# trifectatechfoundation/zlib-rs

Measured on NVIDIA H100. Metric: deflate_level6_raw_input_throughput_silesia_small_tar, higher is better.
Workload: dtype u8

## Files before the change

include/zb_engine.h:

```cpp
#ifndef ZB_ENGINE_H
#define ZB_ENGINE_H
#include <stddef.h>
#include <stdint.h>

#ifdef __cplusplus
extern "C" {
#endif

#define ZB_API __attribute__((visibility("default")))

#define ZB_OK 0
#define ZB_E_NODEVICE (-100)
#define ZB_E_CUDA (-101)
#define ZB_E_BUF (-5)
#define ZB_E_MEM (-4)
#define ZB_E_PARAM (-2)
#define ZB_E_DATA (-3)
#define ZB_E_INTERNAL (-102)

typedef struct zb_engine zb_engine;

typedef struct zb_deflate_result {
    uint64_t out_bytes;
    uint32_t check;
    int32_t data_type;
    uint32_t iterations;
    uint32_t n_symbols;
    uint32_t n_blocks;
    uint32_t gpu_launches;
    int32_t exact_parity;
    float gpu_ms;
    uint32_t bits_used;
    uint32_t carry;
} zb_deflate_result;

ZB_API zb_engine *zb_engine_create(int device, int *err);
ZB_API void zb_engine_destroy(zb_engine *e);
ZB_API const char *zb_last_error(void);
ZB_API int zb_device_count(void);

ZB_API int zb_deflate(zb_engine *e, const void *src, size_t src_len, int src_on_device, void *dst, size_t dst_cap, int dst_on_device,
               int level, int strategy, int window_bits, zb_deflate_result *res);
#define ZB_FLAG_NOT_LAST 1u
#define ZB_FLAG_LOW_PARALLEL 2u
#define ZB_FLAG_CHECK_ADLER 4u
#define ZB_FLAG_CHECK_CRC 8u
#define ZB_FLAG_END_PARTIAL 16u
#define ZB_FLAG_END_BLOCK 32u
#define ZB_FLAG_PRIME(bits, val) ((((uint32_t)(bits) & 7u) << 12) | (((uint32_t)(val) & 0xffu) << 16))
#define ZB_FLAG_MEMLEVEL(m) ((uint32_t)(m) << 8)
ZB_API int zb_deflate_ex(zb_engine *e, const void *src, size_t src_len, int src_on_device, void *dst, size_t dst_cap, int dst_on_device,
                  int level, int strategy, int window_bits, uint32_t flags, zb_deflate_result *res);
ZB_API int zb_deflate_dict(zb_engine *e, const void *dict, size_t dict_len, const void *src, size_t src_len, int src_on_device, void *dst,
                           size_t dst_cap, int dst_on_device, int level, int strategy, int window_bits, uint32_t flags, zb_deflate_result *res);
ZB_API size_t zb_deflate_bound(size_t src_len);

typedef struct zb_inflate_result {
    uint64_t out_bytes;
    uint64_t in_bytes;
    uint32_t check;
    int32_t status;
    uint32_t gpu_launches;
    float gpu_ms;
    char msg[64];
} zb_inflate_result;

ZB_API int zb_inflate(zb_engine *e, const void *src, size_t src_len, int src_on_device, void *dst, size_t dst_cap, int dst_on_device,
               int window_bits, zb_inflate_result *res);

#define ZB_INF_CHECK_ADLER 1u
#define ZB_INF_CHECK_CRC 2u
ZB_API int zb_inflate_ex(zb_engine *e, const void *src, size_t src_len, int src_on_device, void *dst, size_t dst_cap, int dst_on_device,
                         int window_bits, uint32_t flags, zb_inflate_result *res);

typedef struct zb_inflate_seg {
    uint64_t out_bytes;
    uint64_t end_bit;
    uint32_t final_block, need_input, sync_point;
    uint32_t check;
    uint32_t gpu_launches;
    float gpu_ms;
    char msg[64];
} zb_inflate_seg;
ZB_API int zb_inflate_blocks(zb_engine *e, const void *src, size_t src_len, uint64_t start_bit, const void *dict, size_t dict_len,
                             void *dst, size_t dst_cap, int check_kind, uint32_t check_start, zb_inflate_seg *out);

ZB_API int zb_adler32(zb_engine *e, uint32_t start, const void *buf, size_t len, int on_device, uint32_t *out, float *gpu_ms);
ZB_API int zb_crc32(zb_engine *e, uint32_t start, const void *buf, size_t len, int on_device, uint32_t *out, float *gpu_ms);

ZB_API void zb_engine_set_profile(zb_engine *e, int on);
ZB_API int zb_engine_get_profile(zb_engine *e, float *ms, uint32_t *launches, int n);

ZB_API void *zb_device_alloc(zb_engine *e, size_t bytes);
ZB_API void zb_device_free(zb_engine *e, void *p);
ZB_API int zb_copy_to_device(zb_engine *e, void *dst, const void *src, size_t bytes);
ZB_API int zb_copy_to_host(zb_engine *e, void *dst, const void *src, size_t bytes);
ZB_API int zb_device_fill_random(zb_engine *e, void *dst, size_t bytes, uint64_t seed);

#ifdef __cplusplus
}
#endif
#endif
```

zlib_rs_b200/__init__.py:

```python
import ctypes
import os

_HERE = os.path.dirname(os.path.abspath(__file__))
LIB_PATH = os.environ.get("ZB_LIB_PATH") or os.path.join(_HERE, "libz_b200.so")

Z_OK, Z_STREAM_END, Z_NEED_DICT = 0, 1, 2
Z_ERRNO, Z_STREAM_ERROR, Z_DATA_ERROR, Z_MEM_ERROR, Z_BUF_ERROR, Z_VERSION_ERROR = -1, -2, -3, -4, -5, -6
Z_NO_FLUSH, Z_PARTIAL_FLUSH, Z_SYNC_FLUSH, Z_FULL_FLUSH, Z_FINISH, Z_BLOCK = 0, 1, 2, 3, 4, 5
Z_DEFAULT_STRATEGY, Z_FILTERED, Z_HUFFMAN_ONLY, Z_RLE, Z_FIXED = 0, 1, 2, 3, 4
ZLIB_VERSION = b"1.3.0-zlib-rs-0.6.7-b200"
ZB_FLAG_NOT_LAST = 1
ZB_FLAG_LOW_PARALLEL = 2
ZB_FLAG_CHECK_ADLER = 4
ZB_FLAG_CHECK_CRC = 8


class ZStream(ctypes.Structure):
    _fields_ = [("next_in", ctypes.c_void_p), ("avail_in", ctypes.c_uint), ("total_in", ctypes.c_ulong),
                ("next_out", ctypes.c_void_p), ("avail_out", ctypes.c_uint), ("total_out", ctypes.c_ulong),
                ("msg", ctypes.c_char_p), ("state", ctypes.c_void_p), ("zalloc", ctypes.c_void_p),
                ("zfree", ctypes.c_void_p), ("opaque", ctypes.c_void_p), ("data_type", ctypes.c_int),
                ("adler", ctypes.c_ulong), ("reserved", ctypes.c_ulong)]


class DeflateResult(ctypes.Structure):
    _fields_ = [("out_bytes", ctypes.c_uint64), ("check", ctypes.c_uint32), ("data_type", ctypes.c_int32),
                ("iterations", ctypes.c_uint32), ("n_symbols", ctypes.c_uint32), ("n_blocks", ctypes.c_uint32),
                ("gpu_launches", ctypes.c_uint32), ("exact_parity", ctypes.c_int32), ("gpu_ms", ctypes.c_float),
                ("bits_used", ctypes.c_uint32), ("carry", ctypes.c_uint32)]


class InflateResult(ctypes.Structure):
    _fields_ = [("out_bytes", ctypes.c_uint64), ("in_bytes", ctypes.c_uint64), ("check", ctypes.c_uint32),
                ("status", ctypes.c_int32), ("gpu_launches", ctypes.c_uint32), ("gpu_ms", ctypes.c_float),
                ("msg", ctypes.c_char * 64)]


class ZlibError(Exception):
    def __init__(self, code, msg=""):
        super().__init__("zlib error %d %s" % (code, msg))
        self.code = code
        self.msg = msg


_lib = None


def lib():
    global _lib
    if _lib is None:
        if not os.path.exists(LIB_PATH):
            raise RuntimeError("libz_b200.so is not built: run `python -c 'import __graft_entry__ as g; g.build()'` "
                               "or `make -C zlib_rs_b200/csrc` (needs nvcc, sm_90a)")
        L = ctypes.CDLL(LIB_PATH, mode=ctypes.RTLD_LOCAL)
        vp, sz, u32, u64, ci = ctypes.c_void_p, ctypes.c_size_t, ctypes.c_uint32, ctypes.c_uint64, ctypes.c_int
        ul = ctypes.c_ulong
        zs = ctypes.POINTER(ZStream)
        L.zlibVersion.restype = ctypes.c_char_p
        L.zError.restype, L.zError.argtypes = ctypes.c_char_p, [ci]
        L.deflateInit2_.argtypes = [zs, ci, ci, ci, ci, ci, ctypes.c_char_p, ci]
        L.deflateInit_.argtypes = [zs, ci, ctypes.c_char_p, ci]
        L.deflate.argtypes = [zs, ci]
        L.deflateEnd.argtypes = [zs]
        L.deflateReset.argtypes = [zs]
        L.deflateBound.argtypes, L.deflateBound.restype = [zs, ul], ul
        L.inflateInit2_.argtypes = [zs, ci, ctypes.c_char_p, ci]
        L.inflateInit_.argtypes = [zs, ctypes.c_char_p, ci]
        L.inflate.argtypes = [zs, ci]
        L.inflateEnd.argtypes = [zs]
        L.compress2.argtypes = [vp, ctypes.POINTER(ul), vp, ul, ci]
        L.compress.argtypes = [vp, ctypes.POINTER(ul), vp, ul]
        L.compressBound.argtypes, L.compressBound.restype = [ul], ul
        L.uncompress.argtypes = [vp, ctypes.POINTER(ul), vp, ul]
        L.uncompress2.argtypes = [vp, ctypes.POINTER(ul), vp, ctypes.POINTER(ul)]
        for f in ("adler32", "crc32"):
            getattr(L, f).argtypes, getattr(L, f).restype = [ul, vp, ctypes.c_uint], ul
            getattr(L, f + "_z").argtypes, getattr(L, f + "_z").restype = [ul, vp, sz], ul
        L.adler32_combine.argtypes, L.adler32_combine.restype = [ul, ul, ctypes.c_long], ul
        L.crc32_combine.argtypes, L.crc32_combine.restype = [ul, ul, ctypes.c_long], ul
        L.crc32_combine_gen.argtypes, L.crc32_combine_gen.restype = [ctypes.c_long], ul
        L.adler32_combine64.argtypes, L.adler32_combine64.restype = [ul, ul, ctypes.c_longlong], ul
        L.crc32_combine64.argtypes, L.crc32_combine64.restype = [ul, ul, ctypes.c_longlong], ul
        L.crc32_combine_gen64.argtypes, L.crc32_combine_gen64.restype = [ctypes.c_longlong], ul
        L.crc32_combine_op.argtypes, L.crc32_combine_op.restype = [ul, ul, ul], ul
        L.zb_engine_create.argtypes, L.zb_engine_create.restype = [ci, ctypes.POINTER(ci)], vp
        L.zb_engine_destroy.argtypes = [vp]
        L.zb_last_error.restype = ctypes.c_char_p
        L.zb_device_count.restype = ci
        L.zb_deflate.argtypes = [vp, vp, sz, ci, vp, sz, ci, ci, ci, ci, ctypes.POINTER(DeflateResult)]
        L.zb_deflate_ex.argtypes = [vp, vp, sz, ci, vp, sz, ci, ci, ci, ci, u32, ctypes.POINTER(DeflateResult)]
        L.zb_deflate_bound.argtypes, L.zb_deflate_bound.restype = [sz], sz
        L.zb_inflate.argtypes = [vp, vp, sz, ci, vp, sz, ci, ci, ctypes.POINTER(InflateResult)]
        L.zb_adler32.argtypes = [vp, u32, vp, sz, ci, ctypes.POINTER(u32), ctypes.POINTER(ctypes.c_float)]
        L.zb_crc32.argtypes = [vp, u32, vp, sz, ci, ctypes.POINTER(u32), ctypes.POINTER(ctypes.c_float)]
        L.zb_engine_set_profile.argtypes = [vp, ci]
        L.zb_engine_get_profile.argtypes = [vp, ctypes.POINTER(ctypes.c_float), ctypes.POINTER(u32), ci]
        L.zb_device_alloc.argtypes, L.zb_device_alloc.restype = [vp, sz], vp
        L.zb_device_free.argtypes = [vp, vp]
        L.zb_copy_to_device.argtypes = [vp, vp, vp, sz]
        L.zb_copy_to_host.argtypes = [vp, vp, vp, sz]
        L.zb_device_fill_random.argtypes = [vp, vp, sz, u64]
        _lib = L
    return _lib


def _buf(data):
    data = bytes(data)
    return data, (ctypes.c_char * max(len(data), 1)).from_buffer_copy(data or b"\0")


def compressBound(n):
    return lib().compressBound(n)


def compress2(data, level=-1):
    data, src = _buf(data)
    n = ctypes.c_ulong(lib().compressBound(len(data)))
    dst = ctypes.create_string_buffer(n.value)
    rc = lib().compress2(dst, ctypes.byref(n), src, len(data), level)
    if rc != Z_OK:
        raise ZlibError(rc, lib().zb_last_error().decode())
    return dst.raw[: n.value]


def compress(data):
    return compress2(data, -1)


def uncompress(data, bufsize):
    data, src = _buf(data)
    n = ctypes.c_ulong(bufsize)
    dst = ctypes.create_string_buffer(max(bufsize, 1))
    rc = lib().uncompress(dst, ctypes.byref(n), src, len(data))
    if rc != Z_OK:
        raise ZlibError(rc, lib().zb_last_error().decode())
    return dst.raw[: n.value]


def crc32(data, value=0):
    data, src = _buf(data)
    return lib().crc32_z(value, src if data else None, len(data)) if data else (value if True else 0)


def adler32(data, value=1):
    data, src = _buf(data)
    return lib().adler32_z(value, src, len(data)) if data else value


class Deflate:

    def __init__(self, level=-1, window_bits=15, mem_level=8, strategy=0):
        self.s = ZStream()
        rc = lib().deflateInit2_(ctypes.byref(self.s), level, 8, window_bits, mem_level, strategy, ZLIB_VERSION,
                                 ctypes.sizeof(ZStream))
        if rc != Z_OK:
            raise ZlibError(rc, (self.s.msg or b"").decode())
        self._open = True

    def deflate(self, data, flush=Z_NO_FLUSH, out_chunk=1 << 16):
        data, src = _buf(data)
        self.s.next_in = ctypes.addressof(src)
        self.s.avail_in = len(data)
        out = bytearray()
        obuf = ctypes.create_string_buffer(out_chunk)
        while True:
            self.s.next_out = ctypes.addressof(obuf)
            self.s.avail_out = out_chunk
            rc = lib().deflate(ctypes.byref(self.s), flush)
            out += obuf.raw[: out_chunk - self.s.avail_out]
            if rc == Z_STREAM_END:
                break
            if rc == Z_BUF_ERROR and self.s.avail_in == 0:
                break
            if rc != Z_OK:
                raise ZlibError(rc, (self.s.msg or b"").decode())
            if self.s.avail_out != 0 and self.s.avail_in == 0:
                break
        self.last_rc = rc
        return bytes(out)

    @property
    def adler(self):
        return self.s.adler

    @property
    def total_in(self):
        return self.s.total_in

    @property
    def total_out(self):
        return self.s.total_out

    @property
    def data_type(self):
        return self.s.data_type

    def end(self):
        if self._open:
            self._open = False
            return lib().deflateEnd(ctypes.byref(self.s))
        return Z_OK

    def __del__(self):
        try:
            self.end()
        except Exception:
            pass


class Inflate:

    def __init__(self, window_bits=15):
        self.s = ZStream()
        rc = lib().inflateInit2_(ctypes.byref(self.s), window_bits, ZLIB_VERSION, ctypes.sizeof(ZStream))
        if rc != Z_OK:
            raise ZlibError(rc, (self.s.msg or b"").decode())
        self._open = True
        self.eof = False

    def inflate(self, data, flush=Z_NO_FLUSH, out_chunk=1 << 16):
        data, src = _buf(data)
        self.s.next_in = ctypes.addressof(src)
        self.s.avail_in = len(data)
        out = bytearray()
        obuf = ctypes.create_string_buffer(out_chunk)
        while True:
            self.s.next_out = ctypes.addressof(obuf)
            self.s.avail_out = out_chunk
            rc = lib().inflate(ctypes.byref(self.s), flush)
            out += obuf.raw[: out_chunk - self.s.avail_out]
            if rc == Z_STREAM_END:
                self.eof = True
                break
            if rc == Z_BUF_ERROR:
                break
            if rc != Z_OK:
                raise ZlibError(rc, (self.s.msg or b"").decode())
            if self.s.avail_out != 0 and self.s.avail_in == 0:
                break
        self.last_rc = rc
        return bytes(out)

    @property
    def adler(self):
        return self.s.adler

    def end(self):
        if self._open:
            self._open = False
            return lib().inflateEnd(ctypes.byref(self.s))
        return Z_OK

    def __del__(self):
        try:
            self.end()
        except Exception:
            pass


class Engine:
    def __init__(self, device=0):
        err = ctypes.c_int(0)
        self.h = lib().zb_engine_create(device, ctypes.byref(err))
        if not self.h:
            raise RuntimeError("zb_engine_create failed (%d): %s" % (err.value, lib().zb_last_error().decode()))

    def close(self):
        if self.h:
            lib().zb_engine_destroy(self.h)
            self.h = None

    def __del__(self):
        try:
            self.close()
        except Exception:
            pass

    def _check(self, rc):
        if rc != 0:
            raise ZlibError(rc, lib().zb_last_error().decode())

    def alloc(self, n):
        p = lib().zb_device_alloc(self.h, n)
        if not p:
            raise MemoryError("zb_device_alloc(%d)" % n)
        return p

    def free(self, p):
        lib().zb_device_free(self.h, p)

    def to_device(self, dptr, data):
        data, src = _buf(data)
        self._check(lib().zb_copy_to_device(self.h, dptr, src, len(data)))

    def to_host(self, dptr, n):
        dst = ctypes.create_string_buffer(max(n, 1))
        self._check(lib().zb_copy_to_host(self.h, dst, dptr, n))
        return dst.raw[:n]

    def deflate(self, src, n=None, level=6, strategy=0, window_bits=15, flags=0, src_on_device=False, dst=None, dst_cap=0,
                dst_on_device=False, mem_level=8):
        res = DeflateResult()
        flags |= (mem_level & 15) << 8
        keep = None
        if not src_on_device:
            data, keep = _buf(src)
            n = len(data)
            src = ctypes.addressof(keep)
        own = None
        if dst is None:
            dst_cap = lib().zb_deflate_bound(n) + 64
            own = ctypes.create_string_buffer(dst_cap)
            dst = ctypes.addressof(own)
            dst_on_device = False
        rc = lib().zb_deflate_ex(self.h, src, n, int(src_on_device), dst, dst_cap, int(dst_on_device), level, strategy,
                                 window_bits, flags, ctypes.byref(res))
        self._check(rc)
        return (own.raw[: res.out_bytes] if own is not None else None), res

    def inflate(self, src, out_cap, n=None, window_bits=15, src_on_device=False, dst=None, dst_on_device=False):
        res = InflateResult()
        keep = None
        if not src_on_device:
            data, keep = _buf(src)
            n = len(data)
            src = ctypes.addressof(keep)
        own = None
        if dst is None:
            own = ctypes.create_string_buffer(max(out_cap, 1))
            dst = ctypes.addressof(own)
        rc = lib().zb_inflate(self.h, src, n, int(src_on_device), dst, out_cap, int(dst_on_device), window_bits, ctypes.byref(res))
        return rc, (own.raw[: res.out_bytes] if own is not None else None), res

    def adler32(self, buf, n=None, start=1, on_device=False):
        out, ms = ctypes.c_uint32(0), ctypes.c_float(0)
        keep = None
        if not on_device:
            data, keep = _buf(buf)
            n = len(data)
            buf = ctypes.addressof(keep)
        self._check(lib().zb_adler32(self.h, start, buf, n, int(on_device), ctypes.byref(out), ctypes.byref(ms)))
        return out.value, ms.value

    def crc32(self, buf, n=None, start=0, on_device=False):
        out, ms = ctypes.c_uint32(0), ctypes.c_float(0)
        keep = None
        if not on_device:
            data, keep = _buf(buf)
            n = len(data)
            buf = ctypes.addressof(keep)
        self._check(lib().zb_crc32(self.h, start, buf, n, int(on_device), ctypes.byref(out), ctypes.byref(ms)))
        return out.value, ms.value

    PHASES = ["links", "match", "nxt", "path", "emit_holes", "tail", "blocks", "encode", "checksum", "h2d", "d2h", "match_first"]

    def set_profile(self, on=True):
        lib().zb_engine_set_profile(self.h, int(on))

    def get_profile(self):
        ms = (ctypes.c_float * 12)()
        ln = (ctypes.c_uint32 * 12)()
        k = lib().zb_engine_get_profile(self.h, ms, ln, 12)
        return {self.PHASES[i]: {"ms": ms[i], "launches": ln[i]} for i in range(min(k, len(self.PHASES)))}

    def fill_random(self, dptr, n, seed=42):
        self._check(lib().zb_device_fill_random(self.h, dptr, n, seed))
```

zlib_rs_b200/csrc/zb_engine.cu:

```cuda
#include <cuda_runtime.h>
#include <stdio.h>
#include <stdlib.h>
#include <string.h>
#include <new>
#include "../../include/zb_engine.h"
#include "zb_kernels.cuh"
#include "zb_engine_internal.h"

namespace zb {

constexpr uint32_t kSlowSub9 = 24576;
constexpr uint32_t kTailTiles = 2;
constexpr uint32_t kTailSub = 512;

thread_local char g_err[256] = "";

static void set_err(const char *what, cudaError_t e)
{
    snprintf(g_err, sizeof g_err, "%s: %s", what, cudaGetErrorString(e));
}

#define CK(call)                                                  \
    do {                                                          \
        cudaError_t e_ = (call);                                  \
        if (e_ != cudaSuccess) { set_err(#call, e_); return ZB_E_CUDA; } \
    } while (0)

__global__ void k_match(JobBufs);
__global__ void k_skip(JobBufs);
__global__ void k_nxt(JobBufs);
__global__ void k_path_tiles(JobBufs);
__global__ void k_path_chain(JobBufs, uint32_t, uint32_t);
__global__ void k_path_groups(JobBufs, uint32_t, uint32_t, uint4 *, uint32_t *);
__global__ void k_path_chain2(JobBufs, uint32_t, uint32_t, const uint4 *, uint32_t *, uint32_t *);
__global__ void k_path_mark(JobBufs, const uint32_t *, const uint32_t *);
__global__ void k_iter_lists(JobBufs, uint32_t *, uint32_t *, uint32_t);
__global__ void k_emit(JobBufs);
__global__ void k_holes(JobBufs, uint32_t);
__global__ void k_holes_cmp(JobBufs, uint32_t, uint32_t);
__global__ void k_tail(JobBufs);
__global__ void k_block_hist(JobBufs, uint32_t *);
__global__ void k_build_blocks(JobBufs, const uint32_t *);
__global__ void k_scan_blocks(JobBufs);
__global__ void k_encode(JobBufs);
__global__ void k_finish(JobBufs, const uint32_t *);
__global__ void k_literal_syms(JobBufs);
__global__ void k_stored(JobBufs);
__global__ void k_links2_std(JobBufs, uint32_t);
__global__ void k_links2_roll(JobBufs, uint32_t);
__global__ void k_links_fix_std(JobBufs);
__global__ void k_links_fix_roll(JobBufs);
__global__ void k_slow(JobBufs);
__global__ void k_rle(JobBufs);
__global__ void k_emit_slow(JobBufs);
__global__ void k_tail_slow(JobBufs);
__global__ void k_serial_low(JobBufs);
__global__ void k_links_dict_ghost(JobBufs, uint32_t *);
__global__ void k_links_dict_ghost_apply(JobBufs, const uint32_t *);

constexpr uint32_t kMatchSmemBytes = (kWSize + kMatchSub + 512) + (kWSize + kMatchSub) * 2 + ((kWSize + kMatchSub) / 32 + 1) * 4 * 4 + 8192;
constexpr uint32_t kPathSmemBytes = kPathTile * 4 * 3;
constexpr uint32_t kLinks2SmemBytes = 65536 * 2 + kLinkTile * 2 + kLinkTile + 64 + 2048;
constexpr uint32_t kSkipSmemBytes = 2 * kWSize * 2 + 2 * (2 * kWSize / 32) * 4 + 8192 + 64;
constexpr uint32_t kSlowSubMax = 24576;
constexpr uint32_t kSlowSmemBytes = (kWSize + kSlowSubMax + kSlowAhead) * 3;
constexpr uint32_t kChainSmemBytes = kChainChunkTiles * kPathHead * 8;
constexpr uint32_t kChain2MaxSmem = 200 * 1024;
constexpr uint32_t kSerialSmemBytes = (65536 + kWSize) * 2 + 35824 + 16;
constexpr uint32_t kSerialSmemQuick = 65536 * 2 + 65536 + 16;

int Engine::init(int dev)
{
    int n = 0;
    cudaError_t e = cudaGetDeviceCount(&n);
    if (e != cudaSuccess || n == 0) {
        snprintf(g_err, sizeof g_err, "no CUDA device (%s)", e == cudaSuccess ? "count 0" : cudaGetErrorString(e));
        return ZB_E_NODEVICE;
    }
    if (dev < 0 || dev >= n) { snprintf(g_err, sizeof g_err, "device %d out of range", dev); return ZB_E_PARAM; }
    device = dev;
    CK(cudaSetDevice(dev));
    CK(cudaStreamCreateWithFlags(&st, cudaStreamNonBlocking));
    CK(cudaStreamCreateWithFlags(&st2, cudaStreamNonBlocking));
    CK(cudaEventCreateWithFlags(&evf, cudaEventDisableTiming));
    CK(cudaEventCreateWithFlags(&evt, cudaEventDisableTiming));
    for (int i = 0; i < kUpChunks; i++) CK(cudaEventCreateWithFlags(&evc[i], cudaEventDisableTiming));
    CK(cudaEventCreateWithFlags(&evk, cudaEventDisableTiming));
    CK(cudaEventCreate(&ev0));
    CK(cudaEventCreate(&ev1));
    CK(upload_tables());
    CK(cudaFuncSetAttribute(k_match, cudaFuncAttributeMaxDynamicSharedMemorySize, kMatchSmemBytes));
    CK(cudaFuncSetAttribute(k_skip, cudaFuncAttributeMaxDynamicSharedMemorySize, kSkipSmemBytes));
    CK(cudaFuncSetAttribute(k_links2_std, cudaFuncAttributeMaxDynamicSharedMemorySize, kLinks2SmemBytes));
    CK(cudaFuncSetAttribute(k_links2_roll, cudaFuncAttributeMaxDynamicSharedMemorySize, kLinks2SmemBytes));
    CK(cudaFuncSetAttribute(k_slow, cudaFuncAttributeMaxDynamicSharedMemorySize, kSlowSmemBytes));
    CK(cudaFuncSetAttribute(k_path_tiles, cudaFuncAttributeMaxDynamicSharedMemorySize, kPathSmemBytes));
    CK(cudaFuncSetAttribute(k_path_mark, cudaFuncAttributeMaxDynamicSharedMemorySize, kPathSmemBytes));
    CK(cudaFuncSetAttribute(k_path_chain, cudaFuncAttributeMaxDynamicSharedMemorySize, kChainSmemBytes));
    CK(cudaFuncSetAttribute(k_path_groups, cudaFuncAttributeMaxDynamicSharedMemorySize, kChain2MaxSmem));
    CK(cudaFuncSetAttribute(k_path_chain2, cudaFuncAttributeMaxDynamicSharedMemorySize, kChain2MaxSmem));
    CK(cudaFuncSetAttribute(k_serial_low, cudaFuncAttributeMaxDynamicSharedMemorySize, kSerialSmemBytes));
    CK(cudaMallocHost(&h_info, sizeof(JobInfo)));
    CK(cudaMalloc(&d_info, sizeof(JobInfo)));
    CK(cudaMalloc(&d_check, 16));
    { int rc_ = inflate_init(); if (rc_ != ZB_OK) return rc_; }
    return ZB_OK;
}

Engine::~Engine()
{
    if (device < 0) return;
    cudaSetDevice(device);
    for (auto &b : bufs) if (b.p) cudaFree(b.p);
    if (h_stage) cudaFreeHost(h_stage);
    if (h_info) cudaFreeHost(h_info);
    if (d_info) cudaFree(d_info);
    if (d_check) cudaFree(d_check);
    if (ev0) cudaEventDestroy(ev0);
    if (ev1) cudaEventDestroy(ev1);
    if (evf) cudaEventDestroy(evf);
    if (evt) cudaEventDestroy(evt);
    for (int i = 0; i < kUpChunks; i++) if (evc[i]) cudaEventDestroy(evc[i]);
    if (evk) cudaEventDestroy(evk);
    if (st2) cudaStreamDestroy(st2);
    if (st) cudaStreamDestroy(st);
}

void Engine::pbegin()
{
    if (!profile) return;
    if (!pev0) { cudaEventCreate(&pev0); cudaEventCreate(&pev1); }
    cudaEventRecord(pev0, st);
}

void Engine::pend(int phase, uint32_t nlaunch)
{
    if (!profile) return;
    cudaEventRecord(pev1, st);
    cudaEventSynchronize(pev1);
    float ms = 0;
    cudaEventElapsedTime(&ms, pev0, pev1);
    phase_ms[phase] += ms;
    phase_launches[phase] += nlaunch;
}

int Engine::reserve(int slot, size_t bytes, void **out)
{
    Buf &b = bufs[slot];
    if (b.cap < bytes) {
        if (b.p) { cudaFree(b.p); b.p = nullptr; b.cap = 0; }
        size_t want = bytes + (bytes >> 3) + 4096;
        cudaError_t e = cudaMalloc(&b.p, want);
        if (e != cudaSuccess) { set_err("cudaMalloc", e); return ZB_E_MEM; }
        b.cap = want;
    }
    *out = b.p;
    return ZB_OK;
}

int Engine::stage(size_t bytes)
{
    if (h_stage_cap < bytes) {
        if (h_stage) cudaFreeHost(h_stage);
        h_stage = nullptr;
        h_stage_cap = 0;
        cudaError_t e = cudaMallocHost(&h_stage, bytes + (bytes >> 3) + 4096);
        if (e != cudaSuccess) { set_err("cudaMallocHost", e); return ZB_E_MEM; }
        h_stage_cap = bytes + (bytes >> 3) + 4096;
    }
    return ZB_OK;
}

enum { S_IN, S_L, S_HOLES, S_HOLESN, S_M, S_NXT, S_PEXIT, S_PCNT, S_SYMIDX, S_TENTRY, S_TSYMB, S_TDIRTY, S_SYMS, S_SYMB,
       S_BLOCKS, S_SCRATCH, S_FREQ, S_OUT, S_CK, S_INF0, S_INF1, S_PHEAD, S_SK, S_MARKN, S_LLIST, S_LCNT, S_BMAP, S_HDIFF, S_HCOARSE, S_CSTATE, S_LISTS, S_LR, S_LLAST, S_BBASE, S_MCHG, S_GFN, S_KEYS, S_COUNT };
static_assert(S_COUNT <= Engine::kSlots, "slots");

size_t deflate_bound(size_t n)
{
    return n + ((n + 7) >> 3) + ((n + 63) >> 6) + 5 + 18 + 64;
}

int Engine::deflate(const void *src, size_t n_in, bool src_dev, void *dst, size_t dst_cap, bool dst_dev, int level, int strategy,
                    int window_bits, uint32_t flags, zb_deflate_result *res, const void *dict, size_t dict_len)
{
    size_t dstart = 0;
    if (dict_len) {
        if (!dict || window_bits >= 0) { snprintf(g_err, sizeof g_err, "a dictionary needs a raw stream (the caller frames FDICT / DICTID)"); return ZB_E_PARAM; }
        if (dict_len >= 2 * (size_t)kWSize) { dict = static_cast<const uint8_t *>(dict) + (dict_len - kWSize); dict_len = kWSize; }
        dstart = dict_len;
    }
    const size_t n = n_in + dstart;
    int mem_level = (int)((flags >> 8) & 15u);
    if (mem_level == 0) mem_level = 8;
    if (mem_level > 9) return ZB_E_PARAM;
    if (!res || (!src && n) || !dst) return ZB_E_PARAM;
    memset(res, 0, sizeof *res);
    if (n > 0xF0000000ull) { snprintf(g_err, sizeof g_err, "input too large for one job (%zu)", n); return ZB_E_PARAM; }
    if (level == -1) level = 6;
    if (level < 0 || level > 9 || strategy < 0 || strategy > 4) return ZB_E_PARAM;
    uint32_t wrap;
    if (window_bits < 0) { if (window_bits < -15 || window_bits > -8) return ZB_E_PARAM; wrap = 0; }
    else if (window_bits > 15) { if (window_bits < 24 || window_bits > 31) return ZB_E_PARAM; wrap = 2; }
    else { if (window_bits < 8) return ZB_E_PARAM; wrap = 1; }
    const int wb = window_bits < 0 ? -window_bits : window_bits > 15 ? window_bits - 16 : window_bits;
    CK(cudaSetDevice(device));
    const uint32_t N = (uint32_t)n;
    launches = 0;

    JobBufs jb;
    memset(&jb, 0, sizeof jb);
    int rc;
    void *p;
    const size_t npad = (size_t)N + kPad;
    const uint32_t nwords = (N >> 5) + 2;
    const uint32_t nmt = N / kMatchTile + 1, npt = N / kPathTile + 1;
    const bool low_parallel = (flags & ZB_FLAG_LOW_PARALLEL) != 0 || dstart != 0;
    const bool serial_low = (level == 1 || level == 2) && strategy != 2 && strategy != 3 && !low_parallel;
    const uint32_t block_syms = (serial_low && level == 1) ? kBlockSyms : (1u << (mem_level + 6)) - 1u;
    const uint32_t max_blocks = N / block_syms + 2;
    const size_t out_cap = (deflate_bound(n) + 15) & ~(size_t)15;
    if ((rc = stage((size_t)nmt + 64 + ((size_t)N / 512 + 2 + npt + nmt + 8) * 4 + 64)) != ZB_OK) return rc;
    uint8_t *h_dirty = static_cast<uint8_t *>(h_stage);
    uint32_t *h_lists = reinterpret_cast<uint32_t *>(static_cast<uint8_t *>(h_stage) + (((size_t)nmt + 64 + 15) & ~(size_t)15));
#define RES(slot, bytes, field, type)                                   \
    if ((rc = reserve(slot, bytes, &p)) != ZB_OK) return rc;            \
    jb.field = static_cast<type>(p);
    uint8_t *d_in;
    if ((rc = reserve(S_IN, npad + 16, &p)) != ZB_OK) return rc;
    d_in = static_cast<uint8_t *>(p);
    jb.in = d_in;
    jb.N = N;
    jb.start = (uint32_t)dstart;
    jb.nmt = nmt;
    jb.tail_start = N > 2 * kTailZone ? N - kTailZone : 0;
    jb.block_syms = block_syms;
    jb.serial_mode = serial_low ? (uint32_t)level : 0u;
    RES(S_L, npad * 2, L, uint16_t *)
    RES(S_SK, npad * 2, SK, uint16_t *)
    RES(S_HOLES, (size_t)nwords * 4, holes, uint32_t *)
    RES(S_HOLESN, (size_t)nwords * 4, holes_new, uint32_t *)
    RES(S_M, npad * 4, M, uint32_t *)
    RES(S_NXT, ((size_t)N + 16) * 4, nxt, uint32_t *)
    RES(S_PEXIT, ((size_t)N + 16) * 4, pexit, uint32_t *)
    RES(S_PCNT, ((size_t)N + 16) * 4, pcnt, uint32_t *)
    RES(S_SYMIDX, ((size_t)N + 16) * 4, symidx, uint32_t *)
    RES(S_PHEAD, (size_t)npt * kPathHead * 8, phead, uint2 *)
    RES(S_TENTRY, (size_t)npt * 4, tile_entry, uint32_t *)
    RES(S_TSYMB, (size_t)npt * 4, tile_symbase, uint32_t *)
    RES(S_MARKN, (size_t)npt + 16, mark_needed, uint8_t *)
    const uint32_t nlists = npt * (kPathTile / kPathSub);
    RES(S_LLIST, (size_t)nlists * kLongPerSub * 4, long_list, uint32_t *)
    RES(S_LCNT, (size_t)nlists * 4, long_cnt, uint32_t *)
    RES(S_TDIRTY, (size_t)nmt + 16, tile_dirty, uint8_t *)
    RES(S_SYMS, ((size_t)N + 64) * sizeof(Sym), syms, Sym *)
    RES(S_SYMB, 40000 * 4, sym_base, uint32_t *)
    RES(S_BMAP, (size_t)nmt * 8192, bucket_map, uint32_t *)
    RES(S_LR, npad * 2, Lr, uint16_t *)
    RES(S_KEYS, npad * 2, keys, uint16_t *)
    RES(S_LLAST, (size_t)nmt * 65536 * 2, link_last, uint16_t *)
    RES(S_CSTATE, (size_t)(npt + 1) * 16, chain_state, uint4 *)
    uint32_t chainG = 16;
    while ((uint64_t)chainG * chainG < npt) chainG += 8;
    const uint32_t chain_groups = (npt + chainG - 1) / chainG;
    const uint32_t chain2_smem = chainG * kPathHead * 8 + chain_groups * kPathHead * 16 + chainG * 8;
    const bool chain2 = chain2_smem <= kChain2MaxSmem;
    if ((rc = reserve(S_GFN, (size_t)chain_groups * kPathHead * 16 + ((size_t)npt + 4) * 4, &p)) != ZB_OK) return rc;
    uint4 *d_gfn = static_cast<uint4 *>(p);
    uint32_t *d_mark_cnt = reinterpret_cast<uint32_t *>(d_gfn + (size_t)chain_groups * kPathHead);
    uint32_t *d_mark_list = d_mark_cnt + 4;
    auto launch_chain = [&](uint32_t first_tile) {
        if (chain2) {
            k_path_groups<<<chain_groups, 1024, chainG * kPathHead * 8, st>>>(jb, npt, chainG, d_gfn, d_mark_cnt);
            k_path_chain2<<<chain_groups, 1024, chain2_smem, st>>>(jb, npt, chainG, d_gfn, d_mark_list, d_mark_cnt);
            launches++;
        } else k_path_chain<<<1, 1024, kChainSmemBytes, st>>>(jb, npt, first_tile);
    };
    auto launch_mark = [&](uint32_t grid) {
        if (chain2) k_path_mark<<<grid < npt ? grid : npt, 1024, kPathSmemBytes, st>>>(jb, d_mark_list, d_mark_cnt);
        else k_path_mark<<<npt, 1024, kPathSmemBytes, st>>>(jb, nullptr, nullptr);
    };
    uint32_t *d_lists;
    const uint32_t max_list = N / 512 + 2;
    if ((rc = reserve(S_LISTS, ((size_t)max_list + npt + nmt + 8) * 4, &p)) != ZB_OK) return rc;
    d_lists = static_cast<uint32_t *>(p);
    RES(S_HDIFF, (size_t)nwords * 8, hdiff, uint32_t *)
    jb.hdiff_words = nwords;
    RES(S_HCOARSE, (size_t)(N >> 10) + 16, hcoarse, uint8_t *)
    RES(S_MCHG, (((size_t)N >> 8) + 16) * 4 + 64, mchg, uint8_t *)
    RES(S_BLOCKS, (size_t)max_blocks * sizeof(BlockDesc), blocks, BlockDesc *)
    RES(S_BBASE, (size_t)max_blocks * 4, block_base, uint32_t *)
    uint32_t *d_freq;
    if ((rc = reserve(S_FREQ, (size_t)max_blocks * 320 * 4, &p)) != ZB_OK) return rc;
    d_freq = static_cast<uint32_t *>(p);
    uint8_t *d_out;
    if (dst_dev && dst_cap >= out_cap) d_out = static_cast<uint8_t *>(dst);
    else { if ((rc = reserve(S_OUT, out_cap + 16, &p)) != ZB_OK) return rc; d_out = static_cast<uint8_t *>(p); }
    jb.out = d_out;
    jb.out_cap = out_cap;
    void *d_ck;
    const size_t ck_bytes = ((size_t)N / 16384 + 16) * 8;
    if ((rc = reserve(S_CK, ck_bytes, &d_ck)) != ZB_OK) return rc;
#undef RES
    jb.info = d_info;
    jb.level = (uint32_t)level;
    jb.strategy_fixed = strategy == 4;
    const bool lf_zero = strategy >= 2;
    jb.wrap = wrap;
    jb.hdr_len = wrap == 1 ? 2 : wrap == 2 ? 10 : 0;
    jb.huffman_only = strategy == 2 && level != 0;
    jb.not_last = (flags & ZB_FLAG_NOT_LAST) ? 1 : 0;
    jb.end_mode = (flags & ZB_FLAG_END_PARTIAL) ? 1u : (flags & ZB_FLAG_END_BLOCK) ? 2u : 0u;
    jb.prime_bits = (flags >> 12) & 7u;
    if ((jb.end_mode && !jb.not_last) || (jb.prime_bits && wrap != 0)) { snprintf(g_err, sizeof g_err, "END_* needs NOT_LAST, PRIME a raw stream"); return ZB_E_PARAM; }
    if (jb.not_last && (level == 0 || wrap != 0)) { snprintf(g_err, sizeof g_err, "NOT_LAST needs raw deflate and level > 0"); return ZB_E_PARAM; }
    jb.xfl = level == 9 ? 2 : (strategy >= 2 || level < 2) ? 4 : 0;
    int eng_level = level;
    const int wb_eff = wb == 8 ? 9 : wb;
    const bool small_ok = wb_eff < 15 && (uint64_t)N + kMinLookahead <= (1ull << wb_eff);
    bool exact = (wb_eff == 15 || small_ok) && (dstart == 0 || wb_eff == 15);
    jb.cinfo = small_ok ? (uint32_t)(wb_eff - 8) : 7u;
    jb.wsize = kWSize;
    const bool serial_win = wb_eff < 15 && !small_ok && N <= 32000u && level >= 3 && level <= 6 && strategy != 2 && strategy != 3;
    if (serial_win) {
        jb.wsize = 1u << wb_eff;
        jb.cinfo = (uint32_t)(wb_eff - 8);
        jb.tail_start = 0;
        exact = true;
    }
    const bool par_win = wb_eff < 15 && !small_ok && !serial_win && level >= 3 && level <= 6 && strategy != 2 && strategy != 3 && dstart == 0;
    if (par_win) {
        jb.wsize = 1u << wb_eff;
        jb.cinfo = (uint32_t)(wb_eff - 8);
        exact = true;
    }
    const bool slow_win = wb_eff < 15 && !small_ok && dstart == 0 && level != 0 && ((level >= 7 && strategy != 2) || strategy == 3);
    if (slow_win) {
        jb.wsize = 1u << wb_eff;
        jb.cinfo = (uint32_t)(wb_eff - 8);
        exact = true;
    }
    if (wb_eff < 15 && (level == 0 || (strategy == 2 && level != 0) || serial_low)) {
        jb.wsize = 1u << wb_eff;
        jb.cinfo = (uint32_t)(wb_eff - 8);
        exact = true;
    }
    if (level != 0 && !jb.huffman_only) {
        if (level < 3 && !serial_low) { eng_level = 3; exact = exact && strategy == 3; }
        if (strategy == 3) jb.slow_mode = 2;
        else if (level > 6) { jb.slow_mode = 1; jb.sp = slow_params(level); jb.sp.filtered = strategy == 1; jb.sp.wsize = jb.wsize; }
    }
    if (jb.slow_mode) jb.tail_start = N;
    jb.lp = level_params(eng_level);
    if (level != 0 && !jb.huffman_only) jb.level = (uint32_t)level;
    if (lf_zero && !jb.strategy_fixed && !jb.huffman_only) jb.level = 1;

    CK(cudaEventRecord(ev0, st));
    if (profile) { for (int i = 0; i < kPhases; i++) { phase_ms[i] = 0; phase_launches[i] = 0; } }
    uint32_t up_chunks = 0;
    size_t up_len[kUpChunks] = {0};
    const bool chunked_upload = !src_dev && !dstart && n_in >= ((size_t)4 << 20) && level != 0 && !jb.huffman_only &&
                                !jb.serial_mode && jb.slow_mode != 2;
    if (chunked_upload) {
        size_t chunk = (n_in / kUpChunks + kLinkTile - 1) / kLinkTile * kLinkTile;
        if (chunk < (size_t)device_sm_count() * kLinkTile) chunk = (size_t)device_sm_count() * kLinkTile;
        CK(cudaStreamWaitEvent(st2, ev0, 0));
        for (size_t off = 0; off < n_in; off += chunk) {
            const size_t len = n_in - off < chunk ? n_in - off : chunk;
            CK(cudaMemcpyAsync(d_in + off, static_cast<const uint8_t *>(src) + off, len, cudaMemcpyHostToDevice, st2));
            if (off + len == n_in) CK(cudaMemsetAsync(d_in + n, 0, kPad, st2));
            CK(cudaEventRecord(evc[up_chunks], st2));
            up_len[up_chunks++] = off + len;
        }
    } else {
        pbegin();
        if (dstart) CK(cudaMemcpyAsync(d_in, dict, dstart, src_dev ? cudaMemcpyDefault : cudaMemcpyHostToDevice, st));
        if (n_in) CK(cudaMemcpyAsync(d_in + dstart, src, n_in, src_dev ? cudaMemcpyDeviceToDevice : cudaMemcpyHostToDevice, st));
        CK(cudaMemsetAsync(d_in + n, 0, kPad, st));
        pend(9, 0);
    }
    CK(cudaMemsetAsync(d_info, 0, sizeof(JobInfo), st));
    CK(cudaMemsetAsync(d_out, 0, out_cap, st));
    if (jb.prime_bits) {
        h_prime = (uint8_t)((flags >> 16) & ((1u << jb.prime_bits) - 1u));
        CK(cudaMemcpyAsync(d_out, &h_prime, 1, cudaMemcpyHostToDevice, st));
    }
    cudaStream_t st_ck = chunked_upload ? st2 : st;
    pbegin();
    if (wrap == 1 || (wrap == 0 && (flags & ZB_FLAG_CHECK_ADLER))) { CK(launch_adler32(d_in + dstart, n_in, 1, d_ck, ck_bytes, d_check, st_ck)); launches += 2; }
    else if (wrap == 2 || (wrap == 0 && (flags & ZB_FLAG_CHECK_CRC))) { CK(launch_crc32(d_in + dstart, n_in, 0, d_ck, ck_bytes, d_check, st_ck)); launches += 2; }
    else CK(cudaMemsetAsync(d_check, 0, 4, st_ck));
    if (chunked_upload) CK(cudaEventRecord(evk, st2));
    pend(8, 2);

    auto links_tiles = [&](bool roll) {
        uint32_t t_done = 0;
        for (uint32_t k = 0; k < (chunked_upload ? up_chunks : 1u); k++) {
            uint32_t t_hi = nmt;
            if (chunked_upload) {
                cudaStreamWaitEvent(st, evc[k], 0);
                if (k + 1 < up_chunks) t_hi = up_len[k] >= 64 ? (uint32_t)((up_len[k] - 64) / kLinkTile) : 0;
            }
            if (t_hi <= t_done) continue;
            if (roll) k_links2_roll<<<t_hi - t_done, 1024, kLinks2SmemBytes, st>>>(jb, t_done);
            else k_links2_std<<<t_hi - t_done, 1024, kLinks2SmemBytes, st>>>(jb, t_done);
            if (k) launches++;
            t_done = t_hi;
        }
        if (chunked_upload) cudaStreamWaitEvent(st, evk, 0);
    };
    uint32_t iters = 0;
    if (level == 0) {
        const uint32_t nb = n_in == 0 ? 1 : (uint32_t)((n_in + 65534) / 65535);
        k_stored<<<nb, 256, 0, st>>>(jb);
        launches++;
        k_finish<<<1, 32, 0, st>>>(jb, d_check);
        launches++;
    } else {
        if (jb.huffman_only) {
            k_literal_syms<<<(uint32_t)(n_in / 256 + 1), 256, 0, st>>>(jb);
            launches++;
        } else if (jb.serial_mode) {
            iters = 1;
            pbegin();
            k_serial_low<<<1, 32, jb.serial_mode == 2 ? kSerialSmemBytes : kSerialSmemQuick, st>>>(jb);
            launches++;
            pend(1, 1);
        } else {
            CK(cudaMemsetAsync(jb.holes, 0, (size_t)nwords * 4, st));
            CK(cudaMemsetAsync(jb.holes_new, 0, (size_t)nwords * 4, st));
            CK(cudaMemsetAsync(jb.tile_dirty, 1, nmt, st));
            CK(cudaMemsetAsync(jb.tile_entry, 0xee, (size_t)npt * 4, st));
            CK(cudaMemsetAsync(jb.M + N, 0, (size_t)kPad * 4, st));
            CK(cudaMemsetAsync(jb.L + N, 0, (size_t)kPad * 2, st));
            pbegin();
            if (jb.slow_mode == 2) {
            } else if (jb.slow_mode && jb.sp.slow) {
                links_tiles(true);
                k_links_fix_roll<<<N / 256 + 1, 256, 0, st>>>(jb);
                launches += 2;
            } else {
                links_tiles(false);
                k_links_fix_std<<<N / 256 + 1, 256, 0, st>>>(jb);
                launches += 2;
                if (dstart >= 3 && n_in) {
                    uint32_t *d_first = reinterpret_cast<uint32_t *>(d_check) + 2;
                    CK(cudaMemsetAsync(d_first, 0xff, 4, st));
                    k_links_dict_ghost<<<(kMaxDist + 255) / 256, 256, 0, st>>>(jb, d_first);
                    k_links_dict_ghost_apply<<<1, 32, 0, st>>>(jb, d_first);
                    launches += 2;
                }
            }
            if (!jb.slow_mode) CK(cudaMemcpyAsync(jb.Lr, jb.L, npad * 2, cudaMemcpyDeviceToDevice, st));
            pend(0, 1);
            if (jb.slow_mode) {
                if (n_in > 0) {
                    iters = 1;
                    pbegin();
                    if (jb.slow_mode == 2) k_rle<<<(N + 255) / 256, 256, 0, st>>>(jb);
                    else {
                        jb.match_sub = level >= 9 ? kSlowSub9 : level == 8 ? 4096u : 8192u;
                        k_slow<<<(N + jb.match_sub - 1) / jb.match_sub, 1024, (kWSize + jb.match_sub + kSlowAhead) * 3, st>>>(jb);
                    }
                    pend(1, 1);
                    if (profile) phase_ms[11] = phase_ms[1];
                    pbegin();
                    k_path_tiles<<<npt, 1024, kPathSmemBytes, st>>>(jb);
                    launch_chain(0);
                    launch_mark(npt);
                    pend(3, 3);
                    pbegin();
                    k_emit_slow<<<(N + 255) / 256, 256, 0, st>>>(jb);
                    pend(4, 1);
                    launches += 5;
                }
                pbegin();
                k_tail_slow<<<1, 32, 0, st>>>(jb);
                launches++;
                pend(5, 1);
            } else {
            if (jb.tail_start > 0) {
                uint32_t n_dirty = nmt;
                for (;;) {
                    iters++;
                    uint32_t mthreads = 1024;
                    if (iters == 1) jb.match_sub = 4096;
                    else if (n_dirty <= kTailTiles) { jb.match_sub = kTailSub; mthreads = 256; }
                    else {
                        const uint64_t per_cta = (uint64_t)n_dirty * kMatchTile / (4 * (uint64_t)device_sm_count());
                        jb.match_sub = per_cta >= 8192 ? 8192 : per_cta >= 4096 ? 4096 : per_cta >= 2048 ? 2048 : 1024;
                    }
                    uint32_t nsub = (N + jb.match_sub - 1) / jb.match_sub;
                    uint32_t n_ptiles = npt, first_ptile = 0;
                    jb.skip_list = nullptr;
                    jb.nxt_list = nullptr;
                    if (iters > 1) {
                        jb.skip_list = d_lists;
                        jb.nxt_list = d_lists + nmt + 8;
                        n_ptiles = h_info->n_ptiles ? h_info->n_ptiles : 1;
                        first_ptile = h_info->first_ptile;
                        nsub = (n_dirty ? n_dirty : 1) * (kMatchTile / jb.match_sub);
                        if (n_dirty) {
                            pbegin();
                            k_skip<<<n_dirty, 1024, kSkipSmemBytes, st>>>(jb);
                            pend(1, 1);
                            launches++;
                        }
                    }
                    const uint32_t msmem = (kWSize + jb.match_sub + 512) + (kWSize + jb.match_sub) * 2 +
                                           (iters > 1 ? ((kWSize + jb.match_sub) / 32 + 1) * 4 * 4 + 8192 : 64);
                    jb.use_bucket_map = iters > 1;
                    pbegin();
                    k_match<<<nsub, mthreads, msmem, st>>>(jb);
                    pend(1, 1);
                    if (profile && iters == 1) phase_ms[11] = phase_ms[1];
                    pbegin();
                    k_nxt<<<n_ptiles * (kPathTile / 1024), 1024, 0, st>>>(jb);
                    pend(2, 1);
                    pbegin();
                    k_path_tiles<<<n_ptiles, 1024, kPathSmemBytes, st>>>(jb);
                    launch_chain(first_ptile);
                    launch_mark(iters == 1 ? npt : 2 * n_ptiles + 16);
                    pend(3, 3);
                    pbegin();
                    k_holes<<<(nlists * kLongPerSub + 255) / 256, 256, 0, st>>>(jb, nlists);
                    k_holes_cmp<<<(nwords + 255) / 256, 256, 0, st>>>(jb, nwords, nmt);
                    pend(4, 2);
                    launches += 7;
                    k_iter_lists<<<1, 1024, 0, st>>>(jb, d_lists, d_lists + nmt + 8, npt);
                    launches++;
                    CK(cudaMemcpyAsync(h_info, d_info, sizeof(JobInfo), cudaMemcpyDeviceToHost, st));
                    CK(cudaStreamSynchronize(st));
                    if (h_info->error) { snprintf(g_err, sizeof g_err, "engine error flags 0x%x (parse)", h_info->error); return ZB_E_INTERNAL; }
                    if (getenv("ZB_DEBUG")) {
                        static unsigned long long last[3];
                        if (iters == 1) memset(last, 0, sizeof last);
                        const double ctas = (double)(h_info->dbg[0] - last[0]) + 1e-9;
                        fprintf(stderr, "iter %u dirty %u: ctas %llu stage %.1f walk %.1f kcyc/cta, holes_changed %u\n", iters, n_dirty,
                                h_info->dbg[0] - last[0], (h_info->dbg[1] - last[1]) / 1e3 / ctas, (h_info->dbg[2] - last[2]) / 1e3 / ctas,
                                h_info->holes_changed);
                        memcpy(last, h_info->dbg, sizeof last);
                    }
                    if (!h_info->holes_changed) break;
                    n_dirty = h_info->n_dirty;
                    if (iters > N / 257u + 4096u) { snprintf(g_err, sizeof g_err, "hole iteration did not converge"); return ZB_E_INTERNAL; }
                }
            }
            CK(cudaEventRecord(evf, st));
            CK(cudaStreamWaitEvent(st2, evf, 0));
            k_tail<<<1, 32, 0, st2>>>(jb);
            launches++;
            CK(cudaEventRecord(evt, st2));
            if (jb.tail_start > 0) {
                pbegin();
                k_emit<<<(jb.tail_start + 255) / 256, 256, 0, st>>>(jb);
                launches++;
                pend(4, 1);
            }
            pbegin();
            CK(cudaStreamWaitEvent(st, evt, 0));
            pend(5, 1);
            }
        }
        CK(cudaMemcpyAsync(h_info, d_info, sizeof(JobInfo), cudaMemcpyDeviceToHost, st));
        CK(cudaStreamSynchronize(st));
        if (h_info->error) { snprintf(g_err, sizeof g_err, "engine error flags 0x%x (tail)", h_info->error); return ZB_E_INTERNAL; }
        const uint32_t nblocks = h_info->n_blocks;
        if (nblocks == 0 || nblocks > max_blocks) { snprintf(g_err, sizeof g_err, "bad block count %u", nblocks); return ZB_E_INTERNAL; }
        pbegin();
        k_block_hist<<<nblocks, 256, 0, st>>>(jb, d_freq);
        k_build_blocks<<<nblocks, 32, 0, st>>>(jb, d_freq);
        k_scan_blocks<<<1, 256, 0, st>>>(jb);
        pend(6, 3);
        pbegin();
        k_encode<<<nblocks, 1024, 0, st>>>(jb);
        k_finish<<<1, 32, 0, st>>>(jb, d_check);
        pend(7, 2);
        launches += 5;
    }
    CK(cudaMemcpyAsync(h_info, d_info, sizeof(JobInfo), cudaMemcpyDeviceToHost, st));
    CK(cudaStreamSynchronize(st));
    CK(cudaGetLastError());
    if (h_info->error) {
        if (h_info->error & 8u) return ZB_E_BUF;
        snprintf(g_err, sizeof g_err, "engine error flags 0x%x (encode)", h_info->error);
        return ZB_E_INTERNAL;
    }
    const uint64_t out_bytes = h_info->out_bytes;
    if (out_bytes > dst_cap) {
        res->out_bytes = out_bytes;
        return ZB_E_BUF;
    }
    if (d_out != dst) {
        pbegin();
        CK(cudaMemcpyAsync(dst, d_out, out_bytes, dst_dev ? cudaMemcpyDeviceToDevice : cudaMemcpyDeviceToHost, st));
        pend(10, 0);
    }
    CK(cudaEventRecord(ev1, st));
    CK(cudaStreamSynchronize(st));
    float ms = 0;
    CK(cudaEventElapsedTime(&ms, ev0, ev1));
    res->out_bytes = out_bytes;
    res->check = h_info->adler;
    res->data_type = (int32_t)h_info->data_type;
    res->iterations = iters;
    res->n_symbols = h_info->n_syms;
    res->n_blocks = h_info->n_blocks;
    res->gpu_launches = launches;
    res->exact_parity = exact ? 1 : 0;
    res->gpu_ms = ms;
    res->bits_used = (uint32_t)(h_info->total_bits & 7u) ? (uint32_t)(h_info->total_bits & 7u) : 8u;
    if (jb.not_last && jb.end_mode && (h_info->total_bits & 7u)) {
        uint8_t last = 0;
        CK(cudaMemcpy(&last, d_out + out_bytes, 1, cudaMemcpyDeviceToHost));
        res->carry = last & ((1u << (h_info->total_bits & 7u)) - 1u);
    }
    return ZB_OK;
}

int Engine::checksum(bool crc, uint32_t start, const void *buf, size_t len, bool on_dev, uint32_t *out, float *ms_out)
{
    if (!out) return ZB_E_PARAM;
    CK(cudaSetDevice(device));
    int rc;
    void *p;
    const uint8_t *d = static_cast<const uint8_t *>(buf);
    CK(cudaEventRecord(ev0, st));
    if (!on_dev && len) {
        if ((rc = reserve(S_IN, len + 16, &p)) != ZB_OK) return rc;
        CK(cudaMemcpyAsync(p, buf, len, cudaMemcpyHostToDevice, st));
        d = static_cast<const uint8_t *>(p);
    }
    void *d_ck;
    const size_t ck_bytes = (len / 16384 + 16) * 8;
    if ((rc = reserve(S_CK, ck_bytes, &d_ck)) != ZB_OK) return rc;
    if (crc) CK(launch_crc32(d, len, start, d_ck, ck_bytes, d_check, st));
    else CK(launch_adler32(d, len, start, d_ck, ck_bytes, d_check, st));
    launches = 2;
    CK(cudaMemcpyAsync(h_info, d_check, 4, cudaMemcpyDeviceToHost, st));
    CK(cudaEventRecord(ev1, st));
    CK(cudaStreamSynchronize(st));
    *out = *reinterpret_cast<uint32_t *>(h_info);
    if (ms_out) CK(cudaEventElapsedTime(ms_out, ev0, ev1));
    return ZB_OK;
}

__global__ void k_fill_random(uint64_t *dst, uint64_t nwords, uint64_t seed)
{
    for (uint64_t i = blockIdx.x * (uint64_t)blockDim.x + threadIdx.x; i < nwords; i += (uint64_t)gridDim.x * blockDim.x) {
        uint64_t z = (i + seed) * 0x9E3779B97F4A7C15ull;
        z = (z ^ (z >> 30)) * 0xBF58476D1CE4E5B9ull;
        z = (z ^ (z >> 27)) * 0x94D049BB133111EBull;
        dst[i] = z ^ (z >> 31);
    }
}

}

using zb::Engine;

extern "C" {

struct zb_engine { Engine e; };

const char *zb_last_error(void) { return zb::g_err; }

int zb_device_count(void)
{
    int n = 0;
    if (cudaGetDeviceCount(&n) != cudaSuccess) return 0;
    return n;
}

zb_engine *zb_engine_create(int device, int *err)
{
    zb_engine *z = new (std::nothrow) zb_engine;
    int rc = z ? z->e.init(device) : ZB_E_MEM;
    if (err) *err = rc;
    if (rc != ZB_OK) { delete z; return nullptr; }
    return z;
}

void zb_engine_destroy(zb_engine *z) { delete z; }

int zb_deflate(zb_engine *z, const void *src, size_t n, int src_dev, void *dst, size_t cap, int dst_dev, int level, int strategy,
               int window_bits, zb_deflate_result *res)
{
    if (!z) return ZB_E_NODEVICE;
    return z->e.deflate(src, n, src_dev != 0, dst, cap, dst_dev != 0, level, strategy, window_bits, 0, res);
}

int zb_deflate_dict(zb_engine *z, const void *dict, size_t dict_len, const void *src, size_t n, int src_dev, void *dst, size_t cap, int dst_dev,
                    int level, int strategy, int window_bits, uint32_t flags, zb_deflate_result *res)
{
    if (!z) return ZB_E_NODEVICE;
    return z->e.deflate(src, n, src_dev != 0, dst, cap, dst_dev != 0, level, strategy, window_bits, flags, res, dict, dict_len);
}

int zb_deflate_ex(zb_engine *z, const void *src, size_t n, int src_dev, void *dst, size_t cap, int dst_dev, int level, int strategy,
                  int window_bits, uint32_t flags, zb_deflate_result *res)
{
    if (!z) return ZB_E_NODEVICE;
    return z->e.deflate(src, n, src_dev != 0, dst, cap, dst_dev != 0, level, strategy, window_bits, flags, res);
}

size_t zb_deflate_bound(size_t n) { return zb::deflate_bound(n); }

int zb_inflate(zb_engine *z, const void *src, size_t n, int src_dev, void *dst, size_t cap, int dst_dev, int window_bits,
               zb_inflate_result *res)
{
    if (!z) return ZB_E_NODEVICE;
    return z->e.inflate(src, n, src_dev != 0, dst, cap, dst_dev != 0, window_bits, res);
}

int zb_inflate_ex(zb_engine *z, const void *src, size_t n, int src_dev, void *dst, size_t cap, int dst_dev, int window_bits, uint32_t flags,
                  zb_inflate_result *res)
{
    if (!z) return ZB_E_NODEVICE;
    return z->e.inflate(src, n, src_dev != 0, dst, cap, dst_dev != 0, window_bits, res, flags);
}

int zb_inflate_blocks(zb_engine *z, const void *src, size_t n, uint64_t start_bit, const void *dict, size_t dict_len, void *dst, size_t cap,
                      int check_kind, uint32_t check_start, zb_inflate_seg *out)
{
    if (!z) return ZB_E_NODEVICE;
    return z->e.inflate_blocks(src, n, start_bit, dict, dict_len, dst, cap, check_kind, check_start, out);
}

int zb_adler32(zb_engine *z, uint32_t start, const void *buf, size_t len, int on_dev, uint32_t *out, float *ms)
{
    if (!z) return ZB_E_NODEVICE;
    return z->e.checksum(false, start, buf, len, on_dev != 0, out, ms);
}

int zb_crc32(zb_engine *z, uint32_t start, const void *buf, size_t len, int on_dev, uint32_t *out, float *ms)
{
    if (!z) return ZB_E_NODEVICE;
    return z->e.checksum(true, start, buf, len, on_dev != 0, out, ms);
}

void zb_engine_set_profile(zb_engine *z, int on) { if (z) z->e.profile = on != 0; }

int zb_engine_get_profile(zb_engine *z, float *ms, uint32_t *launches, int n)
{
    if (!z) return 0;
    int k = n < Engine::kPhases ? n : Engine::kPhases;
    for (int i = 0; i < k; i++) { if (ms) ms[i] = z->e.phase_ms[i]; if (launches) launches[i] = z->e.phase_launches[i]; }
    return k;
}

void *zb_device_alloc(zb_engine *z, size_t bytes)
{
    if (!z) return nullptr;
    cudaSetDevice(z->e.device);
    void *p = nullptr;
    if (cudaMalloc(&p, bytes + zb::kPad + 16) != cudaSuccess) return nullptr;
    cudaMemset(static_cast<uint8_t *>(p) + bytes, 0, zb::kPad);
    return p;
}

void zb_device_free(zb_engine *z, void *p)
{
    if (!z || !p) return;
    cudaSetDevice(z->e.device);
    cudaFree(p);
}

int zb_copy_to_device(zb_engine *z, void *dst, const void *src, size_t bytes)
{
    if (!z) return ZB_E_NODEVICE;
    cudaSetDevice(z->e.device);
    return cudaMemcpy(dst, src, bytes, cudaMemcpyHostToDevice) == cudaSuccess ? ZB_OK : ZB_E_CUDA;
}

int zb_copy_to_host(zb_engine *z, void *dst, const void *src, size_t bytes)
{
    if (!z) return ZB_E_NODEVICE;
    cudaSetDevice(z->e.device);
    return cudaMemcpy(dst, src, bytes, cudaMemcpyDeviceToHost) == cudaSuccess ? ZB_OK : ZB_E_CUDA;
}

int zb_device_fill_random(zb_engine *z, void *dst, size_t bytes, uint64_t seed)
{
    if (!z) return ZB_E_NODEVICE;
    cudaSetDevice(z->e.device);
    zb::k_fill_random<<<zb::device_sm_count() * 8, 256, 0, z->e.st>>>(static_cast<uint64_t *>(dst), bytes / 8, seed);
    return cudaStreamSynchronize(z->e.st) == cudaSuccess ? ZB_OK : ZB_E_CUDA;
}

}
```

zlib_rs_b200/csrc/zb_engine_internal.h:

```cpp
#pragma once
#include <cuda_runtime.h>
#include <stddef.h>
#include <stdint.h>
#include "../../include/zb_engine.h"
#include "zb_kernels.cuh"

namespace zb {

extern thread_local char g_err[256];
size_t deflate_bound(size_t n);

struct Engine {
    static constexpr int kSlots = 40;
    struct Buf { void *p = nullptr; size_t cap = 0; };
    int device = -1;
    cudaStream_t st = nullptr, st2 = nullptr;
    cudaEvent_t evf = nullptr, evt = nullptr;
    cudaEvent_t ev0 = nullptr, ev1 = nullptr;
    static constexpr int kUpChunks = 8;
    cudaEvent_t evk = nullptr;
    cudaEvent_t evc[kUpChunks] = {nullptr};
    Buf bufs[kSlots];
    void *h_stage = nullptr;
    size_t h_stage_cap = 0;
    JobInfo *h_info = nullptr, *d_info = nullptr;
    uint32_t *d_check = nullptr;
    void *d_inf_state = nullptr, *h_inf_state = nullptr;
    uint32_t launches = 0;
    uint8_t h_prime = 0;
    static constexpr int kPhases = 12;
    bool profile = false;
    float phase_ms[kPhases] = {0};
    uint32_t phase_launches[kPhases] = {0};
    cudaEvent_t pev0 = nullptr, pev1 = nullptr;
    void pbegin();
    void pend(int phase, uint32_t nlaunch);

    int init(int dev);
    int inflate_init();
    ~Engine();
    int reserve(int slot, size_t bytes, void **out);
    int stage(size_t bytes);
    int deflate(const void *src, size_t n, bool src_dev, void *dst, size_t dst_cap, bool dst_dev, int level, int strategy,
                int window_bits, uint32_t flags, zb_deflate_result *res, const void *dict = nullptr, size_t dict_len = 0);
    int inflate(const void *src, size_t n, bool src_dev, void *dst, size_t dst_cap, bool dst_dev, int window_bits,
                zb_inflate_result *res, uint32_t flags = 0);
    int inflate_blocks(const void *src, size_t n, uint64_t start_bit, const void *dict, size_t dict_len, void *dst, size_t dst_cap,
                       int check_kind, uint32_t check_start, zb_inflate_seg *out);
    int checksum(bool crc, uint32_t start, const void *buf, size_t len, bool on_dev, uint32_t *out, float *ms);
};

}
```

zlib_rs_b200/csrc/zb_kernels.cu:

```cuda
#include "zb_kernels.cuh"

namespace zb {

__constant__ HuffTables c_tab;

cudaError_t upload_tables()
{
    HuffTables t;
    init_tables(t);
    return cudaMemcpyToSymbol(c_tab, &t, sizeof t);
}

struct GAcc {
    const uint8_t *data;
    uint32_t N;
    const uint16_t *L;
    const uint32_t *holes;
    const uint32_t *M;
    uint32_t w = kWSize;
    __device__ __forceinline__ uint32_t byte(uint32_t y) const
    {
        while (y >= N) {
            if (y < 2 * w) return 0;
            y -= w;
        }
        return data[y];
    }
    __device__ __forceinline__ uint32_t link(uint32_t y) const { return y + 4 <= N ? L[y] : 0; }
    __device__ __forceinline__ bool inserted(uint32_t y) const { return !((holes[y >> 5] >> (y & 31)) & 1u); }
    __device__ __forceinline__ Match mlook(uint32_t x) const
    {
        uint32_t v = M[x];
        return Match{v >> 16, x - (v & 0xffffu)};
    }
};

struct SAcc {
    const uint8_t *sdata;
    const uint16_t *sL;
    const uint32_t *sholes;
    uint32_t ws;
    __device__ __forceinline__ uint32_t byte(uint32_t y) const { return sdata[y - ws]; }
    __device__ __forceinline__ uint32_t link(uint32_t y) const { return sL[y - ws]; }
    __device__ __forceinline__ bool inserted(uint32_t y) const
    {
        uint32_t i = y - ws;
        return !((sholes[i >> 5] >> (i & 31)) & 1u);
    }
};

struct SAccR {
    const uint8_t *sdata;
    const uint16_t *sL;
    uint32_t ws;
    __device__ __forceinline__ uint32_t byte(uint32_t y) const { return sdata[y - ws]; }
    __device__ __forceinline__ uint32_t link(uint32_t y) const { const uint32_t v = sL[y - ws]; return v == 0xffffu ? 0u : v; }
    __device__ __forceinline__ bool inserted(uint32_t) const { return true; }
};


__device__ __forceinline__ uint32_t lds_u32(const uint32_t *words, uint32_t byte_idx)
{
    const uint32_t w = byte_idx >> 2;
    return __funnelshift_r(words[w], words[w + 1], (byte_idx & 3u) * 8u);
}

constexpr uint32_t kFirstFlag = 0xffffu;

template <bool kRoll>
__device__ __forceinline__ void links2_body(const JobBufs &jb, uint32_t tile0)
{
    const uint32_t tile = tile0 + blockIdx.x;
    extern __shared__ __align__(16) uint8_t smem[];
    constexpr uint32_t kKeys = kRoll ? 32768u : 65536u;
    uint16_t *head = reinterpret_cast<uint16_t *>(smem);
    uint16_t *lists = reinterpret_cast<uint16_t *>(smem + kKeys * 2);
    uint8_t *sd = smem + kKeys * 2 + kLinkTile * 2;
    uint16_t *run = reinterpret_cast<uint16_t *>(smem + kKeys * 2 + kLinkTile * 2 + kLinkTile + 64);
    __shared__ uint16_t c_base[32], c_total[32];
    const uint32_t *words = reinterpret_cast<const uint32_t *>(sd);
    const uint32_t tid = threadIdx.x, lane = tid & 31, warp = tid >> 5;
    const uint32_t N = jb.N, need = kRoll ? 3u : 4u, cap = kRoll ? jb.wsize - 1u : jb.wsize - kMinLookahead;
    const uint32_t ts = tile * kLinkTile;
    const uint32_t te = min(ts + kLinkTile, N);
    const uint32_t tv = N >= need ? min(te, N - need + 1) : ts;
    for (uint32_t i = tid; i < kKeys / 2; i += 1024) reinterpret_cast<uint32_t *>(head)[i] = 0;
    run[tid] = 0;
    {
        const uint4 *src = reinterpret_cast<const uint4 *>(jb.in + ts);
        uint4 *dst = reinterpret_cast<uint4 *>(sd);
        for (uint32_t i = tid; i < (te - ts + 16 + 15) / 16; i += 1024) dst[i] = src[i];
    }
    __syncthreads();
    const uint32_t nv = tv > ts ? tv - ts : 0;
    auto key_of = [&](uint32_t i) -> uint32_t { return kRoll ? hash_roll3(sd[i], sd[i + 1], sd[i + 2]) : hash_u32(lds_u32(words, i)); };
    uint16_t *myrun = run + warp * 32;
    for (uint32_t b = 0; b < 32; b++) {
        const uint32_t i = warp * 1024 + b * 32 + lane;
        const uint32_t key = i < nv ? key_of(i) : 0u;
        const uint32_t c = i < nv ? (key & 31u) : 32u;
        if (!kRoll && i < nv) jb.keys[ts + i] = (uint16_t)key;
        const uint32_t peers = __match_any_sync(0xffffffffu, c);
        if (c < 32u && (peers & ((1u << lane) - 1u)) == 0) myrun[c] += (uint16_t)__popc(peers);
        __syncwarp();
    }
    __syncthreads();
    if (warp == 0) {
        uint32_t tot = 0;
        for (uint32_t w = 0; w < 32; w++) { const uint32_t t = run[w * 32 + lane]; run[w * 32 + lane] = (uint16_t)tot; tot += t; }
        uint32_t incl = tot;
#pragma unroll
        for (int d = 1; d < 32; d <<= 1) { const uint32_t t = __shfl_up_sync(0xffffffffu, incl, d); if (lane >= (uint32_t)d) incl += t; }
        const uint32_t base = incl - tot;
        for (uint32_t w = 0; w < 32; w++) run[w * 32 + lane] += (uint16_t)base;
        c_base[lane] = (uint16_t)base;
        c_total[lane] = (uint16_t)tot;
    }
    __syncthreads();
    for (uint32_t b = 0; b < 32; b++) {
        const uint32_t i = warp * 1024 + b * 32 + lane;
        const uint32_t c = i < nv ? (key_of(i) & 31u) : 32u;
        const uint32_t peers = __match_any_sync(0xffffffffu, c);
        const uint32_t lower = peers & ((1u << lane) - 1u);
        if (c < 32u) {
            const uint32_t at = myrun[c];
            lists[at + __popc(lower)] = (uint16_t)i;
        }
        __syncwarp();
        if (c < 32u && lower == 0) myrun[c] += (uint16_t)__popc(peers);
        __syncwarp();
    }
    __syncthreads();
    {
        const uint32_t lb = c_base[warp], ln = c_total[warp];
        for (uint32_t k = 0; k < ln; k += 32) {
            const bool mine = k + lane < ln;
            const uint32_t m = __ballot_sync(0xffffffffu, mine);
            if (mine) {
                const uint32_t i = lists[lb + k + lane];
                const uint32_t key = key_of(i);
                const uint32_t peers = __match_any_sync(m, key);
                const uint32_t lower = peers & ((1u << lane) - 1u);
                const uint32_t pi = __shfl_sync(m, i, lower ? 31 - __clz(lower) : lane);
                const uint32_t pred = lower ? pi + 1 : head[key];
                uint32_t d = pred ? i + 1 - pred : kFirstFlag;
                if (pred && d > cap) d = 0;
                jb.L[ts + i] = (uint16_t)d;
                if ((peers >> lane) == 1u) head[key] = (uint16_t)(i + 1);
            }
            __syncwarp();
        }
    }
    for (uint32_t x = tv + tid; x < te; x += 1024) jb.L[x] = 0;
    __syncthreads();
    uint4 *out = reinterpret_cast<uint4 *>(jb.link_last + (size_t)tile * kKeys);
    const uint4 *hv = reinterpret_cast<const uint4 *>(head);
    for (uint32_t i = tid; i < kKeys * 2 / 16; i += 1024) out[i] = hv[i];
}

template <bool kRoll>
__device__ __forceinline__ void links_fix_body(const JobBufs &jb)
{
    constexpr uint32_t kKeys = kRoll ? 32768u : 65536u;
    const uint32_t x = blockIdx.x * 256 + threadIdx.x;
    if (x >= jb.N || jb.L[x] != kFirstFlag) return;
    const uint32_t tile = x / kLinkTile, cap = kRoll ? jb.wsize - 1u : jb.wsize - kMinLookahead;
    uint32_t d = 0;
    if (tile > 0) {
        const uint8_t *q = jb.in + x;
        const uint32_t key = kRoll ? hash_roll3(q[0], q[1], q[2])
                                   : hash_u32((uint32_t)q[0] | ((uint32_t)q[1] << 8) | ((uint32_t)q[2] << 16) | ((uint32_t)q[3] << 24));
        const uint32_t last = jb.link_last[(size_t)(tile - 1) * kKeys + key];
        if (last) {
            d = x - ((tile - 1) * kLinkTile + last - 1);
            if (d > cap) d = 0;
        }
    }
    jb.L[x] = (uint16_t)d;
}

__global__ void __launch_bounds__(1024) k_links2_std(JobBufs jb, uint32_t tile0) { links2_body<false>(jb, tile0); }
__global__ void __launch_bounds__(1024) k_links2_roll(JobBufs jb, uint32_t tile0) { links2_body<true>(jb, tile0); }
__global__ void __launch_bounds__(256) k_links_fix_std(JobBufs jb) { links_fix_body<false>(jb); }
__global__ void __launch_bounds__(256) k_links_fix_roll(JobBufs jb) { links_fix_body<true>(jb); }

constexpr uint32_t kSkipSpan = 2 * kWSize;
__global__ void __launch_bounds__(1024) k_skip(JobBufs jb)
{
    extern __shared__ __align__(16) uint8_t smem[];
    uint16_t *sL = reinterpret_cast<uint16_t *>(smem);
    uint32_t *sh = reinterpret_cast<uint32_t *>(smem + kSkipSpan * 2);
    uint32_t *sf = sh + kSkipSpan / 32;
    uint32_t *sbm = sf + kSkipSpan / 32;
    const uint32_t tile = jb.skip_list ? jb.skip_list[blockIdx.x] : blockIdx.x;
    const uint32_t ts = tile * kMatchTile;
    if (ts >= jb.N) return;
    const uint32_t te = min(ts + kMatchTile, jb.N);
    const uint32_t ws = ts >= kWSize ? ts - kWSize : 0;
    const uint32_t span = te - ws, tid = threadIdx.x;
    const uint32_t md = jb.wsize - kMinLookahead;
    {
        const uint4 *ls = reinterpret_cast<const uint4 *>(jb.L + ws);
        uint4 *ld = reinterpret_cast<uint4 *>(sL);
        for (uint32_t i = tid; i < (span + 7) / 8; i += 1024) ld[i] = ls[i];
        for (uint32_t i = tid; i < (span + 31) / 32; i += 1024) sh[i] = jb.holes[(ws >> 5) + i];
        const uint32_t *bm1 = jb.bucket_map + (size_t)tile * 2048, *bm0 = tile ? bm1 - 2048 : bm1;
        for (uint32_t i = tid; i < 2048; i += 1024) sbm[i] = bm0[i] | bm1[i];
    }
    __syncthreads();
    {
        const uint4 *kp = reinterpret_cast<const uint4 *>(jb.keys + ws);
        const uint32_t ngrp = ((span + 31) & ~31u) / 8, ngrp_w = (ngrp + 31) & ~31u;
#pragma unroll 4
        for (uint32_t g = tid; g < ngrp_w; g += 1024) {
            const bool valid = g < ngrp;
            const uint4 kv = valid ? kp[g] : make_uint4(0, 0, 0, 0);
            const uint32_t k[8] = {kv.x & 0xffffu, kv.x >> 16, kv.y & 0xffffu, kv.y >> 16, kv.z & 0xffffu, kv.z >> 16, kv.w & 0xffffu, kv.w >> 16};
            uint32_t b = 0;
#pragma unroll
            for (int j = 0; j < 8; j++) b |= ((sbm[k[j] >> 5] >> (k[j] & 31u)) & 1u) << j;
            b <<= 8 * (tid & 3u);
            b |= __shfl_xor_sync(0xffffffffu, b, 1);
            b |= __shfl_xor_sync(0xffffffffu, b, 2);
            if (valid && (tid & 3u) == 0) sf[g >> 2] = b;
        }
    }
    __syncthreads();
    const uint32_t lane = tid & 31, warp = tid >> 5, nwords = (span + 31) / 32;
    uint32_t nz[2];
#pragma unroll
    for (int h = 0; h < 2; h++) {
        const uint32_t w = warp * 64 + lane + 32 * h;
        nz[h] = __ballot_sync(0xffffffffu, w < nwords && (sh[w] & sf[w]) != 0);
    }
    for (uint32_t round = 0; round < 24; round++) {
        int ch = 0;
#pragma unroll
        for (int h = 0; h < 2; h++) {
            uint32_t m = nz[h];
            while (m) {
                const uint32_t w = warp * 64 + (__ffs(m) - 1) + 32 * h;
                m &= m - 1;
                const uint32_t i = w * 32 + lane;
                const bool on = (((sh[w] & sf[w]) >> lane) & 1u) && i < span;
                for (int rep = 0; rep < 6; rep++) {
                    bool c = false;
                    if (on) {
                        const uint32_t d = sL[i];
                        if (d != 0 && d <= i) {
                            const uint32_t t = i - d;
                            if ((sh[t >> 5] >> (t & 31)) & 1u) {
                                const uint32_t d2 = sL[t];
                                sL[i] = (uint16_t)((d2 == 0 || d + d2 > md) ? 0u : d + d2);
                                c = true;
                            }
                        }
                    }
                    __syncwarp();
                    if (!__any_sync(0xffffffffu, c)) break;
                    ch = 1;
                }
            }
        }
        if (!__syncthreads_or(ch)) break;
    }
    for (uint32_t i = ts - ws + tid; i < span; i += 1024) {
        if (sf[i >> 5] == 0) continue;
        if (!((sf[i >> 5] >> (i & 31)) & 1u)) continue;
        uint32_t d = sL[i];
        if (!((sh[i >> 5] >> (i & 31)) & 1u) && d != 0 && d <= i) {
            const uint32_t t = i - d;
            if ((sh[t >> 5] >> (t & 31)) & 1u) {
                const uint32_t d2 = sL[t];
                d = (d2 == 0 || d + d2 > md) ? 0u : d + d2;
            }
        }
        jb.Lr[ws + i] = (uint16_t)d;
    }
}

constexpr uint32_t kMatchData = kWSize + kMatchSub + 512;
constexpr uint32_t kMatchSmem = kMatchData + (kWSize + kMatchSub) * 2 + ((kWSize + kMatchSub) / 32) * 4;

constexpr uint32_t kBatch = 8;
constexpr uint32_t kBatchCmp = 2;
constexpr uint32_t kWalkBurst = 8;
constexpr uint32_t kCmpBurst = 4;
constexpr uint32_t kCoopCmp = 4;
enum { LS_IDLE = 0, LS_WALK = 1, LS_PEND = 2, LS_DONE = 3, LS_FIN = 4 };

struct DiffMaps {
    const uint32_t *del, *pdel;
    const uint32_t *add, *padd;
    __device__ __forceinline__ static bool any(const uint32_t *b, const uint32_t *p, uint32_t lo, uint32_t hi)
    {
        const uint32_t c_hi = p[hi >> 5] + __popc(b[hi >> 5] & ((1u << (hi & 31)) - 1u));
        const uint32_t c_lo = p[lo >> 5] + __popc(b[lo >> 5] & ((1u << (lo & 31)) - 1u));
        return c_hi != c_lo;
    }
};

__device__ __forceinline__ void sld_u64u(uint32_t a, uint32_t &lo, uint32_t &hi)
{
    const uint32_t al = a & ~3u, sh = (a & 3u) * 8u;
    const uint32_t w0 = sld_u32(al), w1 = sld_u32(al + 4), w2 = sld_u32(al + 8);
    lo = __funnelshift_r(w0, w1, sh);
    hi = __funnelshift_r(w1, w2, sh);
}

__device__ __forceinline__ void match_tile_fast(const JobBufs &jb, const uint8_t *sdata, const uint16_t *sL, const uint32_t *sbm,
                                                const DiffMaps dm, uint32_t ws, uint32_t te, uint32_t *s_next)
{
    const bool filt = jb.use_bucket_map != 0;
    const uint32_t dbase = (uint32_t)__cvta_generic_to_shared(sdata);
    const uint32_t lbase = (uint32_t)__cvta_generic_to_shared(sL);
    const uint32_t N = jb.N, nice = jb.lp.nice, budget = jb.lp.chain;
    const uint32_t md = jb.wsize - kMinLookahead;
    const uint32_t lane = threadIdx.x & 31;
    uint32_t *const Mout = jb.M + ws;
    uint16_t *const RDout = jb.SK + ws;
    uint32_t xr = 0;
    uint32_t cr = 0;
    uint32_t dn = 0;
    uint32_t best = 2, chain = 0, res = 0;
    uint32_t xb = 0;
    uint32_t fbase = 0;
    uint32_t lowr = 0;
    uint32_t clen = 0;
    uint32_t rd = 0;
    uint32_t xw4 = 0;
    uint32_t state = LS_IDLE;
    auto second_look = [&]() -> bool {
        const uint32_t w = sld_u32u((best >= 3u ? fbase - 3u : dbase) + cr) ^ xw4;
        return (best >= 3u ? w : (w & 0x00ffffffu)) == 0u;
    };
    auto load_xw4 = [&]() { xw4 = sld_u32u((best >= 3u ? fbase - 3u : dbase) + xr); };
    for (;;) {
        if (state == LS_WALK) {
            if (chain > kWalkBurst) {
                uint32_t crl = cr - lowr;
                uint32_t fl = fbase + lowr, ll = lbase + 2 * lowr;
                asm volatile("" : "+r"(fl), "+r"(ll));
                bool more = false;
#pragma unroll
                for (uint32_t k = 0; k < kWalkBurst; k++) {
                    const uint32_t fbk = sld_u8(fl + crl);
                    dn = sld_u16(ll + 2 * crl);
                    if (fbk == xb) break;
                    chain--;
                    if ((int32_t)crl < (int32_t)dn) break;
                    crl -= dn;
                    if (k + 1 == kWalkBurst) more = true;
                }
                cr = crl + lowr;
                const uint32_t fb = more ? ~xb : sld_u8(fl + crl);
                if (!more) {
                    if (fb == xb) {
                        if (second_look()) { state = LS_PEND; clen = 0; }
                        else {
                            chain--;
                            if (cr < lowr + dn) { rd = 0xffffu; state = LS_FIN; }
                            else cr -= dn;
                        }
                    }
                    else { rd = 0xffffu; state = LS_FIN; }
                }
            } else {
                const uint32_t fb = sld_u8(fbase + cr);
                dn = sld_u16(lbase + 2 * cr);
                if (fb == xb && second_look()) { state = LS_PEND; clen = 0; }
                else if (--chain == 0) { rd = (xr - cr) | 0x8000u; state = LS_FIN; }
                else if (cr < lowr + dn) { rd = 0xffffu; state = LS_FIN; }
                else cr -= dn;
            }
        }
        const uint32_t m_walk = __ballot_sync(0xffffffffu, state == LS_WALK);
        const uint32_t m_pend = __ballot_sync(0xffffffffu, state == LS_PEND);
        if (m_pend && (__popc(m_pend) >= (int)kBatchCmp || m_walk == 0)) {
            uint32_t len = 0;
            bool resolved = false;
            if (state == LS_PEND) {
                uint32_t pa = dbase + xr + clen, pb = dbase + cr + clen;
#pragma unroll 1
                for (uint32_t k = 0; k < kCmpBurst; k++) {
                    uint32_t a0, a1, b0, b1;
                    sld_u64u(pa, a0, a1);
                    sld_u64u(pb, b0, b1);
                    const uint32_t d0 = a0 ^ b0, d1 = a1 ^ b1;
                    if ((d0 | d1) != 0 || clen + 8 >= kMaxMatch) {
                        len = d0 ? clen + ((__ffs(d0) - 1) >> 3) : d1 ? clen + 4 + ((__ffs(d1) - 1) >> 3) : clen + 8;
                        resolved = true;
                        break;
                    }
                    clen += 8; pa += 8; pb += 8;
                }
            }
            uint32_t m_long = 0;
            if (__popc(m_walk | m_pend) <= kCoopCmp) m_long = __ballot_sync(0xffffffffu, state == LS_PEND && !resolved);
            if (m_long) {
                while (m_long) {
                    const uint32_t src = __ffs(m_long) - 1;
                    m_long &= m_long - 1;
                    const uint32_t cl0 = __shfl_sync(0xffffffffu, clen, src);
                    const uint32_t pa0 = __shfl_sync(0xffffffffu, dbase + xr + clen, src) + 8u * lane;
                    const uint32_t pb0 = __shfl_sync(0xffffffffu, dbase + cr + clen, src) + 8u * lane;
                    uint32_t a0, a1, b0, b1;
                    sld_u64u(pa0, a0, a1);
                    sld_u64u(pb0, b0, b1);
                    const uint32_t d0 = a0 ^ b0, d1 = a1 ^ b1;
                    const uint32_t mm = __ballot_sync(0xffffffffu, (d0 | d1) != 0);
                    const uint32_t first = mm ? __ffs(mm) - 1 : 0u;
                    const uint32_t mine = d0 ? ((__ffs(d0) - 1) >> 3) : 4u + ((__ffs(d1) - 1) >> 3);
                    const uint32_t bo = __shfl_sync(0xffffffffu, mine, first);
                    if (lane == src) { len = mm ? cl0 + 8u * first + bo : cl0 + 256u; resolved = true; }
                }
            }
            if (resolved) {
                if (len > kMaxMatch) len = kMaxMatch;
                state = LS_WALK;
                if (len > best) {
                    best = len;
                    res = (len << 16) | (xr - cr);
                    if (best >= nice) { rd = xr - cr; state = LS_FIN; }
                    else { fbase = dbase + best; xb = sld_u8(fbase + xr); load_xw4(); }
                }
                if (state == LS_WALK) {
                    if (--chain == 0) { rd = (xr - cr) | 0x8000u; state = LS_FIN; }
                    else if (cr < lowr + dn) { rd = 0xffffu; state = LS_FIN; }
                    else cr -= dn;
                }
            }
        }
        if (state == LS_FIN) {
            if (filt && Mout[xr] != res) jb.mchg[(ws + xr) >> 6] = 1;
            Mout[xr] = res; RDout[xr] = (uint16_t)rd; state = LS_IDLE;
        }
        const uint32_t m_idle = __ballot_sync(0xffffffffu, state == LS_IDLE);
        const uint32_t m_busy = __ballot_sync(0xffffffffu, state == LS_WALK || state == LS_PEND);
        if ((m_idle | m_busy) == 0) break;
        if (m_idle == 0) continue;
        if (__popc(m_idle) < (int)kBatch && m_busy != 0) continue;
        {
            uint32_t base = 0;
            const uint32_t leader = __ffs(m_idle) - 1;
            if (lane == leader) base = atomicAdd(s_next, (uint32_t)__popc(m_idle));
            base = __shfl_sync(0xffffffffu, base, leader);
            if (state == LS_IDLE) {
                const uint32_t x = base + __popc(m_idle & ((1u << lane) - 1u));
                if (x >= te) state = LS_DONE;
                else if (x + kMSafe > N) { jb.M[x] = 0; }
                else {
                    xr = x - ws;
                    bool skip = false;
                    if (filt) {
                        const uint32_t h = hash_u32(sld_u32u(dbase + xr));
                        skip = !((sbm[h >> 5] >> (h & 31)) & 1u);
                        if (!skip) {
                            const uint32_t rdo = RDout[xr];
                            const bool on_budget = rdo != 0xffffu && (rdo & 0x8000u);
                            const uint32_t lo = rdo == 0xffffu ? (xr > md ? xr - md : 0u) : xr - (rdo & 0x7fffu);
                            bool redo = DiffMaps::any(dm.del, dm.pdel, lo, xr);
                            if (!redo) {
                                if (on_budget) redo = DiffMaps::any(dm.add, dm.padd, lo, xr);
                                else {
                                    const uint32_t m = Mout[xr];
                                    if (m) { const uint32_t h2 = xr - (m & 0xffffu); redo = (dm.add[h2 >> 5] >> (h2 & 31)) & 1u; }
                                }
                            }
                            if (!redo) redo = sld_u16(lbase + 2 * xr) == md;
                            skip = !redo;
                        }
                    }
                    if (!skip) {
                        const uint32_t d0 = sld_u16(lbase + 2 * xr);
                        lowr = xr > md ? xr - md : 0;
                        if (ws == 0 && lowr == 0) lowr = 1;
                        if (xr < lowr + d0) {
                            if (filt && Mout[xr] != 0) jb.mchg[(ws + xr) >> 6] = 1;
                            Mout[xr] = 0; RDout[xr] = 0xffffu;
                        }
                        else {
                            cr = xr - d0;
                            if (lowr + md == xr) lowr++;
                            best = 2; chain = budget; res = 0;
                            fbase = dbase + 2;
                            xb = sld_u8(fbase + xr);
                            load_xw4();
                            state = LS_WALK;
                        }
                    }
                }
            }
        }
    }
}

__global__ void __launch_bounds__(1024, 2) k_match(JobBufs jb)
{
    extern __shared__ __align__(16) uint8_t smem[];
    __shared__ uint32_t s_next;
    __shared__ __align__(8) unsigned long long s_mbar;
    const uint32_t sub = jb.match_sub;
    const uint32_t per_tile = kMatchTile / sub;
    const uint32_t ts = (jb.skip_list ? jb.skip_list[blockIdx.x / per_tile] * per_tile + blockIdx.x % per_tile : blockIdx.x) * sub;
    if (ts >= jb.N) return;
    {
        const uint32_t t0 = ts / kMatchTile, t1 = (min(ts + sub, jb.N) - 1) / kMatchTile;
        if (!jb.tile_dirty[t0] && !jb.tile_dirty[t1]) return;
    }
    const uint32_t data_bytes = kWSize + sub + 512;
    uint8_t *sdata = smem;
    uint16_t *sL = reinterpret_cast<uint16_t *>(smem + data_bytes);
    uint32_t *sh = reinterpret_cast<uint32_t *>(smem + data_bytes + (kWSize + sub) * 2);
    uint32_t *sbm = sh;
    const uint32_t wmax = (kWSize + sub) / 32 + 1;
    uint32_t *sdel = sbm + 2048, *pdel = sdel + wmax, *sadd = pdel + wmax, *padd = sadd + wmax;
    __shared__ uint32_t s_wsum[32];
    const uint32_t N = jb.N;
    const uint32_t te = min(ts + sub, N);
    const uint32_t ws = ts >= kWSize ? ts - kWSize : 0;
    const uint32_t tid = threadIdx.x, nthr = blockDim.x;
    if (jb.use_bucket_map) {
        const uint32_t mt = ts / kMatchTile;
        const uint32_t *bm1 = jb.bucket_map + (size_t)mt * 2048, *bm0 = mt ? bm1 - 2048 : bm1;
        int hit = 0;
        for (uint32_t x = ts + tid; x < te; x += nthr) {
            const uint8_t *q = jb.in + x;
            const uint32_t h = hash_u32((uint32_t)q[0] | ((uint32_t)q[1] << 8) | ((uint32_t)q[2] << 16) | ((uint32_t)q[3] << 24));
            if (((bm0[h >> 5] | bm1[h >> 5]) >> (h & 31)) & 1u) {
                const uint32_t rd = jb.SK[x];
                const uint32_t lo = rd == 0xffffu ? (x > jb.wsize - kMinLookahead ? x - (jb.wsize - kMinLookahead) : 0u) : x - (rd & 0x7fffu);
                for (uint32_t b = lo >> 10; b <= (x >> 10); b++) hit |= jb.hcoarse[b];
            }
        }
        if (!__syncthreads_or(hit)) return;
        for (uint32_t i = tid; i < 2048; i += nthr) sbm[i] = bm0[i] | bm1[i];
        const uint32_t nwd = (te - ws + 31) / 32;
        const uint32_t per = (nwd + 1 + nthr - 1) / nthr;
        const uint32_t wb = tid * per;
        const uint32_t lane_ = tid & 31, warp_ = tid >> 5;
        for (int which = 0; which < 2; which++) {
            const uint32_t *src = which ? jb.hdiff : jb.hdiff + jb.hdiff_words;
            uint32_t *bits = which ? sadd : sdel, *pre = which ? padd : pdel;
            uint32_t mine = 0;
            for (uint32_t k = 0; k < per; k++) {
                const uint32_t w = wb + k;
                if (w <= nwd) { const uint32_t v = w < nwd ? src[(ws >> 5) + w] : 0u; bits[w] = v; mine += __popc(v); }
            }
            uint32_t incl = mine;
#pragma unroll
            for (int d = 1; d < 32; d <<= 1) {
                const uint32_t t = __shfl_up_sync(0xffffffffu, incl, d);
                if (lane_ >= (uint32_t)d) incl += t;
            }
            __syncthreads();
            if (lane_ == 31) s_wsum[warp_] = incl;
            __syncthreads();
            uint32_t run = incl - mine;
            for (uint32_t k = 0; k < warp_; k++) run += s_wsum[k];
            for (uint32_t k = 0; k < per; k++) {
                const uint32_t w = wb + k;
                if (w <= nwd) { pre[w] = run; run += __popc(bits[w]); }
            }
        }
    }
    if (tid == 0) {
        s_next = ts;
        const uint32_t mb = (uint32_t)__cvta_generic_to_shared(&s_mbar);
        asm volatile("mbarrier.init.shared::cta.b64 [%0], 1;" ::"r"(mb) : "memory");
        asm volatile("fence.proxy.async.shared::cta;" ::: "memory");
    }
    const long long t_0 = clock64();
    __syncthreads();
    {
        uint32_t n16 = (te + 512 - ws + 15) / 16;
        if (n16 > data_bytes / 16) n16 = data_bytes / 16;
        const bool bulk = (reinterpret_cast<uintptr_t>(jb.in) & 15u) == 0;
        if (bulk) {
            if (tid == 0) {
                const uint32_t mb = (uint32_t)__cvta_generic_to_shared(&s_mbar), dsts = (uint32_t)__cvta_generic_to_shared(sdata);
                asm volatile("mbarrier.arrive.expect_tx.shared::cta.b64 _, [%0], %1;" ::"r"(mb), "r"(n16 * 16u) : "memory");
                asm volatile("cp.async.bulk.shared::cluster.global.mbarrier::complete_tx::bytes [%0], [%1], %2, [%3];"
                             ::"r"(dsts), "l"(jb.in + ws), "r"(n16 * 16u), "r"(mb) : "memory");
            }
        } else {
            const uint4 *src = reinterpret_cast<const uint4 *>(jb.in + ws);
            uint4 *dst = reinterpret_cast<uint4 *>(sdata);
            for (uint32_t i = tid; i < n16; i += nthr) dst[i] = src[i];
        }
        const uint32_t nl = (te - ws + 7) / 8;
        const uint4 *ls = reinterpret_cast<const uint4 *>(jb.Lr + ws);
        uint4 *ld = reinterpret_cast<uint4 *>(sL);
        for (uint32_t i = tid; i < nl; i += nthr) {
            uint4 v = ls[i];
            v.x |= __vcmpeq2(v.x, 0u); v.y |= __vcmpeq2(v.y, 0u); v.z |= __vcmpeq2(v.z, 0u); v.w |= __vcmpeq2(v.w, 0u);
            ld[i] = v;
        }
        if (bulk) {
            const uint32_t mb = (uint32_t)__cvta_generic_to_shared(&s_mbar);
            uint32_t done = 0;
            while (!done) {
                asm volatile("{\n.reg .pred p;\nmbarrier.try_wait.parity.shared::cta.b64 p, [%1], 0;\nselp.u32 %0, 1, 0, p;\n}"
                             : "=r"(done) : "r"(mb) : "memory");
            }
        }
    }
    __syncthreads();
    const long long t_1 = clock64();
    const LevelParams lp = jb.lp;
    if (!lp.early_exit) {
        match_tile_fast(jb, sdata, sL, sbm, DiffMaps{sdel, pdel, sadd, padd}, ws, te, &s_next);
        __syncthreads();
        if (tid == 0) {
            const long long t_2 = clock64();
            atomicAdd(&jb.info->dbg[0], 1ull);
            atomicAdd(&jb.info->dbg[1], (unsigned long long)(t_1 - t_0));
            atomicAdd(&jb.info->dbg[2], (unsigned long long)(t_2 - t_1));
        }
        return;
    }
    SAccR a{sdata, sL, ws};
    for (uint32_t x = ts + tid; x < te; x += nthr) {
        uint32_t v = 0;
        if (jb.use_bucket_map && x + 4 <= N) {
            const uint32_t h = hash_u32(a.byte(x) | (a.byte(x + 1) << 8) | (a.byte(x + 2) << 16) | (a.byte(x + 3) << 24));
            if (!((sbm[h >> 5] >> (h & 31)) & 1u)) continue;
        }
        if (x + kMSafe <= N) {
            Match m = jb.wsize == kWSize ? lm_walk(a, x, 0xffffffffu, lp) : lm_walk(a, x, 0xffffffffu, lp, DynWin{jb.wsize});
            if (m.len) v = (m.len << 16) | (x - m.start);
        }
        if (jb.use_bucket_map && jb.M[x] != v) jb.mchg[x >> 6] = 1;
        jb.M[x] = v;
        jb.SK[x] = 0xffffu;
    }
}

constexpr uint32_t kMacroReach = 22016;

__device__ __forceinline__ bool path_tile_dirty(const JobBufs &jb, uint32_t pt)
{
    const uint32_t m0 = (pt * kPathTile) / kMatchTile;
    uint32_t m1 = ((pt + 1) * kPathTile + kMacroReach - 1) / kMatchTile;
    if (m1 >= jb.nmt) m1 = jb.nmt - 1;
    bool d = false;
    for (uint32_t m = m0; m <= m1; m++) d = d || jb.tile_dirty[m];
    return d;
}

__global__ void __launch_bounds__(1024) k_nxt(JobBufs jb)
{
    constexpr uint32_t per = kPathTile / 1024;
    const uint32_t tile = jb.nxt_list ? jb.nxt_list[blockIdx.x / per] : blockIdx.x / per;
    if (!path_tile_dirty(jb, tile)) return;
    const uint32_t p = tile * kPathTile + (blockIdx.x % per) * 1024 + threadIdx.x;
    if (p >= jb.tail_start) return;
    if (jb.use_bucket_map) {
        const uint32_t old = jb.nxt[p];
        const uint32_t b0 = p >> 6, b1 = min(p + (old & 0xffffu), jb.N) >> 6;
        bool chg = false;
        for (uint32_t b = b0; b <= b1; b++) chg = chg || jb.mchg[b];
        if (!chg) return;
    }
    GAcc a{jb.in, jb.N, jb.L, jb.holes, jb.M, jb.wsize};
    const uint32_t long_len = 16 * jb.lp.lazy;
    uint32_t ns = 0, nlong = 0, lpos = 0, llen = 0;
    auto see = [&](const Sym &s) {
        if (s.dist && (uint32_t)s.lc + 3u > long_len) { nlong++; lpos = s.pos; llen = s.lc + 3u; }
    };
    const uint32_t np = jb.wsize == kWSize ? macro_step(a, p, jb.lp, jb.tail_start, see, &ns)
                                           : macro_step(a, p, jb.lp, jb.tail_start, see, &ns, DynWin{jb.wsize});
    const uint32_t delta = np - p;
    if (delta > 0xffffu || ns > 0xffu || delta == 0) atomicOr(&jb.info->error, 1u);
    if (nlong && (nlong != 1 || lpos + llen != np || (jb.lp.early_exit ? lpos != p : (llen != 257u && llen != 258u))))
        atomicOr(&jb.info->error, 16u);
    jb.nxt[p] = (delta & 0xffffu) | ((ns & 0xffu) << 16) | (nlong ? kNxtLong : 0u) | (llen == 258u ? kNxtLong258 : 0u) |
                (np >= jb.tail_start ? kNxtTail : 0u);
}

constexpr uint32_t kStuck = 0x80000000u;
__device__ __forceinline__ void path_subtile(const uint32_t *nx, uint32_t *ex, uint32_t *cn, uint32_t s0, uint32_t s1, uint32_t lane)
{
    for (int32_t b = (int32_t)s1 - 32; b >= (int32_t)s0; b -= 32) {
        const uint32_t p = (uint32_t)b + lane;
        const uint32_t v = nx[p];
        uint32_t t, c;
        if (v & kNxtTail) { t = kStuck | p; c = 0; }
        else { t = p + (v & 0xffffu); c = (v >> 16) & 0xffu; }
#pragma unroll
        for (int r = 0; r < 5; r++) {
            const bool inb = !(t & kStuck) && t < (uint32_t)b + 32u;
            const uint32_t src = inb ? t - (uint32_t)b : lane;
            const uint32_t t2 = __shfl_sync(0xffffffffu, t, src);
            const uint32_t c2 = __shfl_sync(0xffffffffu, c, src);
            if (inb) { t = t2; c += c2; }
        }
        if (!(t & kStuck) && t < s1) { c += cn[t]; t = ex[t]; }
        ex[p] = t;
        cn[p] = c;
        __syncwarp();
    }
}

constexpr uint32_t kPathSmem = kPathTile * 4 * 3;

__device__ __forceinline__ void path_load(const JobBufs &jb, uint32_t tbeg, uint32_t *nx)
{
    const uint4 *src = reinterpret_cast<const uint4 *>(jb.nxt + tbeg);
    uint4 *dst = reinterpret_cast<uint4 *>(nx);
#pragma unroll 4
    for (uint32_t g = threadIdx.x; g < kPathTile / 4; g += blockDim.x) {
        const uint32_t p = tbeg + 4 * g;
        uint4 v;
        if (p + 3 < jb.tail_start) v = src[g];
        else {
            const uint32_t t = kNxtTail | 1u;
            v.x = p < jb.tail_start ? jb.nxt[p] : t;
            v.y = p + 1 < jb.tail_start ? jb.nxt[p + 1] : t;
            v.z = p + 2 < jb.tail_start ? jb.nxt[p + 2] : t;
            v.w = t;
        }
        dst[g] = v;
    }
}

__global__ void __launch_bounds__(1024) k_path_tiles(JobBufs jb)
{
    extern __shared__ __align__(16) uint8_t smem[];
    uint32_t *nx = reinterpret_cast<uint32_t *>(smem);
    uint32_t *ex = nx + kPathTile;
    uint32_t *cn = ex + kPathTile;
    const uint32_t tile = jb.nxt_list ? jb.nxt_list[blockIdx.x] : blockIdx.x;
    const uint32_t tbeg = tile * kPathTile;
    if (!path_tile_dirty(jb, tile)) return;
    path_load(jb, tbeg, nx);
    __syncthreads();
    const uint32_t warp = threadIdx.x >> 5, lane = threadIdx.x & 31;
    constexpr uint32_t kExitSub = 1024, nsub = kPathTile / kExitSub;
    for (uint32_t s = warp; s < nsub; s += blockDim.x / 32) path_subtile(nx, ex, cn, s * kExitSub, (s + 1) * kExitSub, lane);
    __syncthreads();
    for (int32_t j = (int32_t)nsub - 2; j >= 0; j--) {
        for (uint32_t i = threadIdx.x; i < kExitSub; i += blockDim.x) {
            const uint32_t p = (uint32_t)j * kExitSub + i;
            uint32_t t = ex[p];
            if (!(t & kStuck) && t < kPathTile) { cn[p] += cn[t]; ex[p] = ex[t]; }
        }
        __syncthreads();
    }
    for (uint32_t i = threadIdx.x; i < kPathTile; i += blockDim.x) {
        const uint32_t p = tbeg + i;
        const uint32_t t = ex[i];
        const uint32_t xa = (t & kStuck) ? (kStuck | (tbeg + (t & ~kStuck))) : tbeg + t;
        if (p < jb.tail_start) {
            jb.pexit[p] = xa;
            jb.pcnt[p] = cn[i];
        }
        if (i < kPathHead) jb.phead[(size_t)tile * kPathHead + i] = make_uint2(xa, cn[i]);
    }
}

constexpr uint32_t kChainChunk = kChainChunkTiles;
__global__ void __launch_bounds__(1024) k_path_chain(JobBufs jb, uint32_t ntiles, uint32_t first_tile)
{
    extern __shared__ __align__(16) uint8_t smem[];
    uint2 *hd = reinterpret_cast<uint2 *>(smem);
    __shared__ uint32_t s_e, s_base, s_done, s_tail;
    __shared__ uint32_t c_entry[kChainChunk], c_base[kChainChunk];
    if (threadIdx.x == 0) {
        if (first_tile == 0) { s_e = jb.start; s_base = 0; s_done = jb.tail_start == 0; s_tail = jb.start; }
        else { const uint4 v = jb.chain_state[first_tile]; s_e = v.x; s_base = v.y; s_done = v.z; s_tail = v.w; }
    }
    for (uint32_t t = threadIdx.x; t < first_tile; t += blockDim.x) jb.mark_needed[t] = 0;
    __syncthreads();
    for (uint32_t c0 = first_tile; c0 < ntiles; c0 += kChainChunk) {
        const uint32_t nt = min(kChainChunk, ntiles - c0);
        for (uint32_t i = threadIdx.x; i < nt * kPathHead; i += blockDim.x) hd[i] = jb.phead[(size_t)c0 * kPathHead + i];
        __syncthreads();
        if (threadIdx.x == 0) {
            uint32_t e = s_e, base = s_base;
            bool done = s_done != 0;
            uint32_t tail_entry = s_tail;
            for (uint32_t k = 0; k < nt; k++) {
                const uint32_t tbeg = (c0 + k) * kPathTile, tend = tbeg + kPathTile;
                jb.chain_state[c0 + k] = make_uint4(e, base, done ? 1u : 0u, tail_entry);
                c_base[k] = base;
                if (done || e >= tend || e >= jb.tail_start) { c_entry[k] = 0xffffffffu; continue; }
                c_entry[k] = e;
                uint32_t x, c;
                if (e - tbeg < kPathHead) { const uint2 v = hd[k * kPathHead + (e - tbeg)]; x = v.x; c = v.y; }
                else { x = jb.pexit[e]; c = jb.pcnt[e]; }
                base += c;
                if (x & kStuck) { tail_entry = x & ~kStuck; done = true; }
                else e = x;
            }
            s_e = e; s_base = base; s_done = done; s_tail = tail_entry;
        }
        __syncthreads();
        for (uint32_t k = threadIdx.x; k < nt; k += blockDim.x) {
            const uint32_t t = c0 + k;
            jb.tile_symbase[t] = c_base[k];
            jb.mark_needed[t] = (jb.tile_entry[t] != c_entry[k]) || path_tile_dirty(jb, t);
            jb.tile_entry[t] = c_entry[k];
        }
        __syncthreads();
    }
    if (threadIdx.x == 0) {
        uint32_t tail_entry = s_tail;
        if (!s_done) { tail_entry = s_e; if (s_e < jb.tail_start) atomicOr(&jb.info->error, 2u); }
        jb.info->tail_entry = tail_entry;
        jb.info->n_mid_syms = s_base;
    }
}

struct ChainState { uint32_t e, base, done, tail; };

template <bool OUT>
__device__ __forceinline__ void chain_walk_group(const JobBufs &jb, const uint2 *hd, uint32_t t0, uint32_t nt, ChainState &s,
                                                 uint32_t *c_entry, uint32_t *c_base)
{
    for (uint32_t k = 0; k < nt; k++) {
        const uint32_t tbeg = (t0 + k) * kPathTile, tend = tbeg + kPathTile;
        if (OUT) c_base[k] = s.base;
        if (s.done || s.e >= tend || s.e >= jb.tail_start) { if (OUT) c_entry[k] = 0xffffffffu; continue; }
        if (OUT) c_entry[k] = s.e;
        uint32_t x, c;
        if (s.e - tbeg < kPathHead) { const uint2 v = hd[k * kPathHead + (s.e - tbeg)]; x = v.x; c = v.y; }
        else { x = jb.pexit[s.e]; c = jb.pcnt[s.e]; }
        s.base += c;
        if (x & kStuck) { s.tail = x & ~kStuck; s.done = 1; }
        else s.e = x;
    }
}

__device__ __forceinline__ void chain_stage_heads(const JobBufs &jb, uint2 *hd, uint32_t t0, uint32_t nt)
{
    const uint4 *src = reinterpret_cast<const uint4 *>(jb.phead + (size_t)t0 * kPathHead);
    uint4 *dst = reinterpret_cast<uint4 *>(hd);
    for (uint32_t i = threadIdx.x; i < nt * kPathHead / 2; i += blockDim.x) dst[i] = src[i];
}

__global__ void __launch_bounds__(1024) k_path_groups(JobBufs jb, uint32_t ntiles, uint32_t G, uint4 *gfn, uint32_t *mark_cnt)
{
    if (blockIdx.x == 0 && threadIdx.x == 0) *mark_cnt = 0;
    extern __shared__ __align__(16) uint8_t smem[];
    uint2 *hd = reinterpret_cast<uint2 *>(smem);
    const uint32_t t0 = blockIdx.x * G, nt = min(G, ntiles - t0);
    chain_stage_heads(jb, hd, t0, nt);
    __syncthreads();
    if (threadIdx.x < kPathHead) {
        ChainState s{t0 * kPathTile + threadIdx.x, 0u, 0u, 0u};
        chain_walk_group<false>(jb, hd, t0, nt, s, nullptr, nullptr);
        gfn[(size_t)blockIdx.x * kPathHead + threadIdx.x] = make_uint4(s.e, s.base, s.done, s.tail);
    }
}

__global__ void __launch_bounds__(1024) k_path_chain2(JobBufs jb, uint32_t ntiles, uint32_t G, const uint4 *gfn, uint32_t *mark_list,
                                                        uint32_t *mark_cnt)
{
    extern __shared__ __align__(16) uint8_t smem[];
    uint2 *hd = reinterpret_cast<uint2 *>(smem);
    uint4 *sg = reinterpret_cast<uint4 *>(smem + (size_t)G * kPathHead * 8);
    uint32_t *c_entry = reinterpret_cast<uint32_t *>(sg + (size_t)blockIdx.x * kPathHead), *c_base = c_entry + G;
    __shared__ ChainState s_st;
    __shared__ uint32_t s_j;
    const uint32_t g = blockIdx.x;
    for (uint32_t i = threadIdx.x; i < g * kPathHead; i += blockDim.x) sg[i] = gfn[i];
    if (threadIdx.x == 0) { s_st = ChainState{jb.start, 0u, jb.tail_start == 0 ? 1u : 0u, jb.start}; s_j = 0; }
    __syncthreads();
    for (;;) {
        if (threadIdx.x == 0) {
            ChainState s = s_st;
            uint32_t j = s_j;
            for (; j < g; j++) {
                const uint32_t gbeg = j * G * kPathTile;
                if (s.done || s.e >= jb.tail_start || s.e - gbeg >= G * kPathTile) continue;
                if (s.e - gbeg >= kPathHead) break;
                const uint4 f = sg[j * kPathHead + (s.e - gbeg)];
                s.e = f.x; s.base += f.y;
                if (f.z) { s.done = 1; s.tail = f.w; }
            }
            s_st = s; s_j = j;
        }
        __syncthreads();
        const uint32_t j = s_j;
        if (j >= g) break;
        chain_stage_heads(jb, hd, j * G, G);
        __syncthreads();
        if (threadIdx.x == 0) {
            ChainState s = s_st;
            chain_walk_group<false>(jb, hd, j * G, G, s, nullptr, nullptr);
            s_st = s; s_j = j + 1;
        }
        __syncthreads();
    }
    const uint32_t t0 = g * G, nt = min(G, ntiles - t0);
    chain_stage_heads(jb, hd, t0, nt);
    __syncthreads();
    if (threadIdx.x == 0) {
        ChainState s = s_st;
        chain_walk_group<true>(jb, hd, t0, nt, s, c_entry, c_base);
        if (g == gridDim.x - 1) {
            uint32_t tail_entry = s.tail;
            if (!s.done) { tail_entry = s.e; if (s.e < jb.tail_start) atomicOr(&jb.info->error, 2u); }
            jb.info->tail_entry = tail_entry;
            jb.info->n_mid_syms = s.base;
        }
    }
    __syncthreads();
    for (uint32_t k = threadIdx.x; k < nt; k += blockDim.x) {
        const uint32_t t = t0 + k;
        jb.tile_symbase[t] = c_base[k];
        const bool mn = (jb.tile_entry[t] != c_entry[k]) || path_tile_dirty(jb, t);
        jb.mark_needed[t] = mn;
        jb.tile_entry[t] = c_entry[k];
        if (mn) mark_list[atomicAdd(mark_cnt, 1u)] = t;
    }
}

__global__ void __launch_bounds__(1024) k_path_mark(JobBufs jb, const uint32_t *list, const uint32_t *list_cnt)
{
    extern __shared__ __align__(16) uint8_t smem[];
    uint32_t *nx = reinterpret_cast<uint32_t *>(smem);
    uint32_t *ex = nx + kPathTile;
    uint32_t *cn = ex + kPathTile;
    __shared__ uint32_t sub_entry[kPathTile / kPathSub], sub_base[kPathTile / kPathSub];
    constexpr uint32_t nsub = kPathTile / kPathSub;
    const uint32_t count = list ? *list_cnt : gridDim.x;
    for (uint32_t b = blockIdx.x; b < count; b += gridDim.x) {
        const uint32_t tile = list ? list[b] : b;
        const uint32_t tbeg = tile * kPathTile;
        if (!jb.mark_needed[tile]) continue;
        const uint32_t entry = jb.tile_entry[tile];
        if (threadIdx.x < nsub) jb.long_cnt[tile * nsub + threadIdx.x] = 0;
        if (entry == 0xffffffffu) {
            for (uint32_t i = threadIdx.x; i < kPathTile; i += blockDim.x)
                if (tbeg + i < jb.tail_start) jb.symidx[tbeg + i] = 0;
            continue;
        }
        __syncthreads();
        path_load(jb, tbeg, nx);
        __syncthreads();
        const uint32_t warp = threadIdx.x >> 5, lane = threadIdx.x & 31;
        for (uint32_t s = warp; s < nsub; s += blockDim.x / 32) path_subtile(nx, ex, cn, s * kPathSub, (s + 1) * kPathSub, lane);
        __syncthreads();
        if (threadIdx.x == 0) {
            uint32_t cur = entry - tbeg, cbase = 0;
            for (uint32_t j = 0; j < nsub; j++) {
                if (!(cur & kStuck) && cur < (j + 1) * kPathSub) {
                    sub_entry[j] = cur;
                    sub_base[j] = cbase;
                    cbase += cn[cur];
                    cur = ex[cur];
                } else sub_entry[j] = 0xffffffffu;
            }
        }
        __syncthreads();
        for (uint32_t i = threadIdx.x; i < kPathTile; i += blockDim.x) ex[i] = 0;
        __syncthreads();
        if (threadIdx.x < nsub) {
            const uint32_t s = threadIdx.x;
            uint32_t p = sub_entry[s];
            if (p != 0xffffffffu) {
                uint32_t idx = sub_base[s], nlong = 0;
                const uint32_t s1 = (s + 1) * kPathSub;
                uint32_t *ll = jb.long_list + (size_t)(tile * nsub + s) * kLongPerSub;
                while (p < s1) {
                    const uint32_t v = nx[p];
                    if (v & kNxtTail) break;
                    if (v & kNxtLong) {
                        if (nlong < kLongPerSub) ll[nlong++] = tbeg + p;
                        else atomicOr(&jb.info->error, 32u);
                    }
                    ex[p] = idx + 1;
                    idx += (v >> 16) & 0xffu;
                    p += v & 0xffffu;
                }
                jb.long_cnt[tile * nsub + s] = nlong;
            }
        }
        __syncthreads();
        for (uint32_t i = threadIdx.x; i < kPathTile; i += blockDim.x)
            if (tbeg + i < jb.tail_start) jb.symidx[tbeg + i] = ex[i];
    }
}

__global__ void __launch_bounds__(256) k_holes(JobBufs jb, uint32_t nlists)
{
    const uint32_t t = blockIdx.x * blockDim.x + threadIdx.x;
    {
        const uint32_t nthr = gridDim.x * blockDim.x;
        for (uint32_t i = t; i < jb.nmt; i += nthr) jb.tile_dirty[i] = 0;
        for (uint32_t i = t; i < jb.nmt * 512; i += nthr) reinterpret_cast<uint4 *>(jb.bucket_map)[i] = make_uint4(0, 0, 0, 0);
        for (uint32_t i = t; i < (jb.N >> 10) + 16; i += nthr) jb.hcoarse[i] = 0;
        for (uint32_t i = t; i < (jb.N >> 8) + 16; i += nthr) reinterpret_cast<uint32_t *>(jb.mchg)[i] = 0;
        if (t == 0) jb.info->holes_changed = 0;
    }
    const uint32_t list = t / kLongPerSub, slot = t % kLongPerSub;
    if (list >= nlists || slot >= jb.long_cnt[list]) return;
    const uint32_t p = jb.long_list[(size_t)list * kLongPerSub + slot];
    const uint32_t v = jb.nxt[p], delta = v & 0xffffu;
    const uint32_t len = jb.lp.early_exit ? delta : ((v & kNxtLong258) ? 258u : 257u);
    const uint32_t pos = p + delta - len;
    uint32_t y0 = pos + 1, y1 = pos + len - 1;
    uint32_t *hn = jb.holes_new;
    while (y0 < y1) {
        const uint32_t w = y0 >> 5, lo = y0 & 31;
        const uint32_t n = min(32u - lo, y1 - y0);
        const uint32_t mask = (n == 32 ? 0xffffffffu : ((1u << n) - 1u)) << lo;
        atomicOr(&hn[w], mask);
        y0 += n;
    }
}

__global__ void __launch_bounds__(256) k_emit(JobBufs jb)
{
    const uint32_t p = blockIdx.x * blockDim.x + threadIdx.x;
    if (p >= jb.tail_start) return;
    const uint32_t idx = jb.symidx[p];
    if (!idx) return;
    GAcc a{jb.in, jb.N, jb.L, jb.holes, jb.M, jb.wsize};
    uint32_t k = jb.tile_symbase[p / kPathTile] + idx - 1, ns = 0;
    Sym *syms = jb.syms;
    auto put = [&](const Sym &s) { syms[k++] = s; };
    if (jb.wsize == kWSize) macro_step(a, p, jb.lp, jb.tail_start, put, &ns);
    else macro_step(a, p, jb.lp, jb.tail_start, put, &ns, DynWin{jb.wsize});
}

__global__ void __launch_bounds__(256) k_holes_cmp(JobBufs jb, uint32_t nwords, uint32_t nmtiles)
{
    __shared__ uint32_t sb[2048];
    const uint32_t w = blockIdx.x * blockDim.x + threadIdx.x;
    uint32_t a = 0, b = 0;
    if (w < nwords) { a = jb.holes[w]; b = jb.holes_new[w]; }
    const bool changed = a != b;
    if (!__syncthreads_or(changed)) {
        if (w < nwords) { jb.hdiff[w] = 0; jb.hdiff[jb.hdiff_words + w] = 0; jb.holes_new[w] = 0; }
        return;
    }
    for (uint32_t i = threadIdx.x; i < 2048; i += blockDim.x) sb[i] = 0;
    __syncthreads();
    if (w < nwords) {
        jb.hdiff[w] = b & ~a;
        jb.hdiff[jb.hdiff_words + w] = a & ~b;
        if (changed) {
            jb.hcoarse[w >> 5] = 1;
            const uint32_t t = (w * 32) / kMatchTile;
            jb.info->holes_changed = 1u;
            jb.tile_dirty[t] = 1;
            if (t + 1 < nmtiles) jb.tile_dirty[t + 1] = 1;
            jb.holes[w] = b;
            uint32_t diff = a ^ b;
            while (diff) {
                const uint32_t y = w * 32 + (__ffs(diff) - 1);
                diff &= diff - 1;
                if (y + 4 <= jb.N) {
                    const uint8_t *q = jb.in + y;
                    const uint32_t h = hash_u32((uint32_t)q[0] | ((uint32_t)q[1] << 8) | ((uint32_t)q[2] << 16) | ((uint32_t)q[3] << 24));
                    atomicOr(&sb[h >> 5], 1u << (h & 31));
                }
            }
        }
        jb.holes_new[w] = 0;
    }
    __syncthreads();
    uint32_t *bm = jb.bucket_map + (size_t)((blockIdx.x * blockDim.x * 32) / kMatchTile) * 2048;
    for (uint32_t i = threadIdx.x; i < 2048; i += blockDim.x) if (sb[i]) atomicOr(&bm[i], sb[i]);
}

__global__ void __launch_bounds__(1024) k_iter_lists(JobBufs jb, uint32_t *skip_list, uint32_t *path_list, uint32_t npt)
{
    __shared__ uint32_t s_wsum[32], s_total, s_first;
    const uint32_t tid = threadIdx.x, lane = tid & 31, warp = tid >> 5;
    if (tid == 0) s_first = 0xffffffffu;
    uint32_t base = 0;
    for (int which = 0; which < 2; which++) {
        const uint32_t n = which ? npt : jb.nmt;
        uint32_t *out = which ? path_list : skip_list;
        base = 0;
        for (uint32_t c0 = 0; c0 < n; c0 += 1024) {
            const uint32_t i = c0 + tid;
            const bool d = i < n && (which ? path_tile_dirty(jb, i) : jb.tile_dirty[i] != 0);
            const uint32_t m = __ballot_sync(0xffffffffu, d);
            __syncthreads();
            if (lane == 0) s_wsum[warp] = __popc(m);
            __syncthreads();
            if (warp == 0) {
                const uint32_t v = s_wsum[lane];
                uint32_t incl = v;
#pragma unroll
                for (int k = 1; k < 32; k <<= 1) { const uint32_t t = __shfl_up_sync(0xffffffffu, incl, k); if (lane >= (uint32_t)k) incl += t; }
                s_wsum[lane] = incl - v;
                if (lane == 31) s_total = incl;
            }
            __syncthreads();
            if (d) {
                out[base + s_wsum[warp] + __popc(m & ((1u << lane) - 1u))] = i;
                if (which) atomicMin(&s_first, i);
            }
            base += s_total;
        }
        __syncthreads();
        if (tid == 0) {
            if (which) { jb.info->n_ptiles = base; jb.info->first_ptile = s_first == 0xffffffffu ? 0u : s_first; }
            else jb.info->n_dirty = base;
        }
        if (tid == 0 && base == 0) out[0] = 0;
    }
}

struct GAccW {
    GAcc g;
    uint32_t w;
    __device__ __forceinline__ uint32_t byte(uint32_t y) const
    {
        while (y >= g.N) {
            if (y < 2 * w) return 0;
            y -= w;
        }
        return g.data[y];
    }
    __device__ __forceinline__ uint32_t link(uint32_t y) const { return g.link(y); }
    __device__ __forceinline__ bool inserted(uint32_t y) const { return g.inserted(y); }
};

__global__ void __launch_bounds__(32) k_tail(JobBufs jb)
{
    __shared__ uint32_t ins[1024];
    if (threadIdx.x != 0) return;
    GAcc a{jb.in, jb.N, jb.L, jb.holes, jb.M, jb.wsize};
    const uint32_t p0 = max(jb.info->tail_entry, jb.start);
    const uint32_t n_mid = jb.info->n_mid_syms;
    uint32_t k = 0;
    Sym *syms = jb.syms + n_mid;
    uint32_t *sb = jb.sym_base;
    if (jb.N - p0 > 1024u * 32u - 64u) { atomicOr(&jb.info->error, 4u); return; }
    auto emit = [&](const Sym &s, uint32_t B) {
        syms[k] = s;
        sb[k] = B;
        k++;
    };
    uint32_t fb;
    if (jb.wsize == kWSize) fb = serial_medium(a, jb.N, p0, ins, 1024u, jb.lp, emit);
    else fb = serial_medium(GAccW{a, jb.wsize}, jb.N, p0, ins, 1024u, jb.lp, emit, DynWin{jb.wsize});
    jb.info->n_syms = n_mid + k;
    jb.info->final_base = fb;
    jb.info->n_blocks = (n_mid + k) / jb.block_syms + 1;
}

__device__ __forceinline__ uint32_t sym_end(const Sym &s) { return s.pos + (s.dist ? (uint32_t)s.lc + 3u : 1u); }

__global__ void __launch_bounds__(256) k_block_hist(JobBufs jb, uint32_t *freq )
{
    __shared__ uint32_t lf[kLCodes], df[kDCodes];
    const uint32_t b = blockIdx.x;
    const uint32_t nsyms = jb.info->n_syms, nblocks = jb.info->n_blocks;
    for (uint32_t i = threadIdx.x; i < kLCodes; i += blockDim.x) lf[i] = 0;
    if (threadIdx.x < kDCodes) df[threadIdx.x] = 0;
    __syncthreads();
    const uint32_t begin = b * jb.block_syms;
    const uint32_t count = (b + 1 < nblocks) ? jb.block_syms : nsyms - begin;
    for (uint32_t i = threadIdx.x; i < count; i += blockDim.x) {
        const Sym s = jb.syms[begin + i];
        if (s.dist == 0) atomicAdd(&lf[s.lc], 1u);
        else {
            atomicAdd(&lf[257 + c_tab.length_code[s.lc]], 1u);
            atomicAdd(&df[d_code(c_tab, s.dist - 1u)], 1u);
        }
    }
    __syncthreads();
    for (uint32_t i = threadIdx.x; i < kLCodes; i += blockDim.x) freq[b * 320 + i] = lf[i];
    if (threadIdx.x < kDCodes) freq[b * 320 + kLCodes + threadIdx.x] = df[threadIdx.x];
    if (threadIdx.x == 0) {
        BlockDesc &bd = jb.blocks[b];
        const bool last = b + 1 == nblocks;
        bd.sym_begin = begin;
        bd.sym_count = count;
        bd.last = last && !jb.not_last;
        const uint32_t start = begin == 0 ? jb.start : sym_end(jb.syms[begin - 1]);
        const uint32_t end = last ? jb.N : sym_end(jb.syms[begin + count - 1]);
        bd.in_start = start;
        bd.in_len = end - start;
        uint32_t Bf;
        if (last) Bf = jb.info->final_base;
        else {
            const uint32_t li = begin + count - 1, n_mid = jb.info->n_mid_syms;
            if (jb.serial_mode) {
                Bf = jb.serial_mode == 2 ? jb.block_base[b] : 0;
            } else if (jb.huffman_only) {
                const uint32_t q = jb.syms[li].pos, w = jb.wsize;
                Bf = q < 2 * w ? 0 : w * (1 + (q - 2 * w) / w);
            } else if (jb.slow_mode == 2) {
                Bf = base_at(jb.syms[li].pos, jb.N, jb.wsize);
            } else if (jb.slow_mode) {
                Bf = base_at(jb.syms[li].pos + 1, jb.N, jb.wsize);
            } else Bf = li < n_mid ? wbase_w(DynWin{jb.wsize}, jb.syms[li].pos) : jb.sym_base[li - n_mid];
        }
        bd.have_window = start >= Bf;
    }
}

__device__ __forceinline__ uint32_t brev_bits(uint32_t code, uint32_t len) { return __brev(code) >> (32u - len); }

template <int KIND>
__device__ __forceinline__ uint32_t xbits_of(uint32_t n) { return KIND == 0 ? (n >= 257 ? extra_lbits(n - 257) : 0u) : KIND == 1 ? extra_dbits(n) : extra_blbits(n); }

template <int KIND>
__device__ int build_tree_warp(TreeScratch &s, TreeState &st, CtData *tree, uint32_t *sh_cnt )
{
    constexpr int elems = KIND == 0 ? kLCodes : KIND == 1 ? kDCodes : kBlCodes;
    constexpr int max_length = KIND == 2 ? kMaxBlBits : kMaxBits;
    const uint32_t lane = threadIdx.x & 31;
    int heap_len = 0, max_code = -1;
    for (int b0 = 0; b0 < elems; b0 += 32) {
        const int n = b0 + (int)lane;
        const bool nz = n < elems && tree[n].fc != 0;
        const uint32_t m = __ballot_sync(0xffffffffu, nz);
        if (nz) { s.heap[heap_len + 1 + __popc(m & ((1u << lane) - 1u))] = (uint32_t)n; s.depth[n] = 0; }
        else if (n < elems) tree[n].dl = 0;
        heap_len += __popc(m);
        if (m) max_code = b0 + 31 - __clz(m);
    }
    __syncwarp();
    if (heap_len < 2) {
        if (lane == 0) {
            while (heap_len < 2) {
                const int node = max_code < 2 ? ++max_code : 0;
                s.heap[++heap_len] = (uint32_t)node;
                tree[node].fc = 1;
                s.depth[node] = 0;
                st.opt_len--;
                if (KIND == 0) st.static_len -= c_tab.sl_len[node];
                else if (KIND == 1) st.static_len -= 5;
            }
        }
        heap_len = 2;
        max_code = __shfl_sync(0xffffffffu, max_code, 0);
        __syncwarp();
    }
    for (int n = 1 + (int)lane; n <= heap_len; n += 32) s.hk[n] = heap_entry(tree, s.depth, s.heap[n]);
    __syncwarp();
    for (int lvl = 31 - __clz(heap_len / 2); lvl >= 0; lvl--) {
        const int first = 1 << lvl, last = min((2 << lvl) - 1, heap_len / 2);
        for (int k = first + (int)lane; k <= last; k += 32) pqdownheap(s, heap_len, k);
        __syncwarp();
    }
    int heap_max = kHeapSize;
    if (lane == 0) {
        int node = elems;
        do {
            const int n = (int)(s.hk[1] & 0xffffu);
            s.hk[1] = s.hk[heap_len--];
            pqdownheap(s, heap_len, 1);
            const int m = (int)(s.hk[1] & 0xffffu);
            s.heap[--heap_max] = (uint32_t)n;
            s.heap[--heap_max] = (uint32_t)m;
            tree[node].fc = (uint16_t)(tree[n].fc + tree[m].fc);
            s.depth[node] = (uint8_t)((s.depth[n] >= s.depth[m] ? s.depth[n] : s.depth[m]) + 1);
            tree[n].dl = tree[m].dl = (uint16_t)node;
            s.hk[1] = heap_entry(tree, s.depth, (uint32_t)node);
            node++;
            pqdownheap(s, heap_len, 1);
        } while (heap_len >= 2);
        s.heap[--heap_max] = (uint32_t)(s.hk[1] & 0xffffu);
        int overflow = 0;
        tree[s.heap[heap_max]].dl = 0;
        for (int h = heap_max + 1; h < kHeapSize; h++) {
            const int n = (int)s.heap[h];
            int bits = tree[tree[n].dl].dl + 1;
            if (bits > max_length) { bits = max_length; overflow++; }
            tree[n].dl = (uint16_t)bits;
        }
        sh_cnt[0] = (uint32_t)overflow;
    }
    heap_max = __shfl_sync(0xffffffffu, heap_max, 0);
    __syncwarp();
    const int overflow = (int)sh_cnt[0];
    __syncwarp();
    if (lane < 16) sh_cnt[lane] = 0;
    __syncwarp();
    uint64_t opt = 0, stat = 0;
    for (int n = (int)lane; n <= max_code; n += 32) {
        const uint32_t bits = tree[n].dl;
        if (tree[n].fc == 0 || bits == 0) continue;
        atomicAdd(&sh_cnt[bits], 1u);
        const uint32_t xb = xbits_of<KIND>((uint32_t)n);
        const uint64_t f = tree[n].fc;
        opt += f * (uint64_t)(bits + xb);
        if (KIND == 0) stat += f * (uint64_t)(c_tab.sl_len[n] + xb);
        else if (KIND == 1) stat += f * (uint64_t)(5 + xb);
    }
#pragma unroll
    for (int d = 16; d >= 1; d >>= 1) { opt += __shfl_xor_sync(0xffffffffu, opt, d); stat += __shfl_xor_sync(0xffffffffu, stat, d); }
    __syncwarp();
    if (lane == 0) {
        st.opt_len += opt;
        st.static_len += stat;
        if (overflow > 0) {
            int ov = overflow, bits;
            do {
                bits = max_length - 1;
                while (sh_cnt[bits] == 0) bits--;
                sh_cnt[bits]--;
                sh_cnt[bits + 1] += 2;
                sh_cnt[max_length]--;
                ov -= 2;
            } while (ov > 0);
            int h = kHeapSize;
            for (bits = max_length; bits != 0; bits--) {
                int n = (int)sh_cnt[bits];
                while (n != 0) {
                    const int m = (int)s.heap[--h];
                    if (m > max_code) continue;
                    if (tree[m].dl != (uint16_t)bits) {
                        st.opt_len += (uint64_t)bits * tree[m].fc;
                        st.opt_len -= (uint64_t)tree[m].dl * tree[m].fc;
                        tree[m].dl = (uint16_t)bits;
                    }
                    n--;
                }
            }
        }
    }
    __syncwarp();
    uint32_t nc = 0;
    {
        uint32_t code = 0;
        for (uint32_t b = 1; b <= (uint32_t)kMaxBits; b++) { code = (code + sh_cnt[b - 1]) << 1; if (b == lane) nc = code; }
    }
    for (int b0 = 0; b0 <= max_code; b0 += 32) {
        const int n = b0 + (int)lane;
        const uint32_t len = n <= max_code ? tree[n].dl : 0u;
        const uint32_t same = __match_any_sync(0xffffffffu, len);
        const uint32_t rank = __popc(same & ((1u << lane) - 1u));
        const uint32_t base = __shfl_sync(0xffffffffu, nc, len & 31u);
        if (len) tree[n].fc = (uint16_t)brev_bits(base + rank, len);
#pragma unroll 1
        for (uint32_t l = 1; l <= (uint32_t)kMaxBits; l++) {
            const uint32_t cnt = __popc(__ballot_sync(0xffffffffu, len == l));
            if (lane == l) nc += cnt;
        }
    }
    __syncwarp();
    return max_code;
}

struct WordSink {
    uint8_t *buf;
    uint32_t nbits;
    __device__ __forceinline__ void put(uint32_t val, uint32_t len)
    {
        const uint32_t byte = nbits >> 3, sh = nbits & 7u;
        const uint32_t v = (val & ((1u << len) - 1u)) << sh;
        if (sh == 0) buf[byte] = (uint8_t)v; else buf[byte] |= (uint8_t)v;
        if (sh + len > 8) { buf[byte + 1] = (uint8_t)(v >> 8); if (sh + len > 16) buf[byte + 2] = (uint8_t)(v >> 16); }
        nbits += len;
    }
};

__device__ void send_tree_fast(WordSink &o, const CtData *bltree, const CtData *tree, int max_code)
{
    int prevlen = -1, curlen, nextlen = tree[0].dl, count = 0, max_count = 7, min_count = 4;
    if (nextlen == 0) { max_count = 138; min_count = 3; }
    for (int n = 0; n <= max_code; n++) {
        curlen = nextlen;
        nextlen = tree[n + 1].dl;
        if (++count < max_count && curlen == nextlen) continue;
        else if (count < min_count) { do { o.put(bltree[curlen].fc, bltree[curlen].dl); } while (--count != 0); }
        else if (curlen != 0) {
            if (curlen != prevlen) { o.put(bltree[curlen].fc, bltree[curlen].dl); count--; }
            o.put(bltree[16].fc, bltree[16].dl);
            o.put((uint32_t)(count - 3), 2);
        } else if (count <= 10) {
            o.put(bltree[17].fc, bltree[17].dl);
            o.put((uint32_t)(count - 3), 3);
        } else {
            o.put(bltree[18].fc, bltree[18].dl);
            o.put((uint32_t)(count - 11), 7);
        }
        count = 0;
        prevlen = curlen;
        if (nextlen == 0) { max_count = 138; min_count = 3; }
        else if (curlen == nextlen) { max_count = 6; min_count = 3; }
        else { max_count = 7; min_count = 4; }
    }
}

__device__ void build_block_warp(TreeScratch &s, BlockDesc &b, const uint32_t *lfreq, const uint32_t *dfreq, bool have_window,
                                 bool strategy_fixed, uint32_t *sh_cnt, TreeState *sh_st)
{
    const uint32_t lane = threadIdx.x & 31;
    uint64_t opt_lenb = 0, static_lenb = 0;
    int max_blindex = 0, lmax = 0, dmax = 0;
    TreeState &st = *sh_st;
    if (lane == 0) { st = TreeState{0, 0}; b.data_type = 2; b.no_eob = 0; }
    __syncwarp();
    if (b.sym_count == 0) {
        if (lane == 0) st.static_len = 7;
    } else {
        {
            bool black = false, white = false;
            for (uint32_t n = lane; n < 256; n += 32) {
                if (lfreq[n] == 0) continue;
                if (n < 32 && ((0xf3ffc07fu >> n) & 1u)) black = true;
                if (n == 9 || n == 10 || n == 13 || n >= 32) white = true;
            }
            const bool ab = __any_sync(0xffffffffu, black), aw = __any_sync(0xffffffffu, white);
            if (lane == 0) b.data_type = ab ? 0u : aw ? 1u : 0u;
        }
        for (int n = (int)lane; n < kHeapSize; n += 32) s.ltree[n] = CtData{(uint16_t)(n < kLCodes ? lfreq[n] : 0), 0};
        for (int n = (int)lane; n < 2 * kDCodes + 1; n += 32) s.dtree[n] = CtData{(uint16_t)(n < kDCodes ? dfreq[n] : 0), 0};
        for (int n = (int)lane; n < 2 * kBlCodes + 1; n += 32) s.bltree[n] = CtData{0, 0};
        __syncwarp();
        if (lane == 0) s.ltree[kEndBlock].fc = 1;
        __syncwarp();
        lmax = build_tree_warp<0>(s, st, s.ltree, sh_cnt);
        dmax = build_tree_warp<1>(s, st, s.dtree, sh_cnt);
        if (lane == 0) {
            scan_tree(s.bltree, s.ltree, lmax);
            scan_tree(s.bltree, s.dtree, dmax);
        }
        __syncwarp();
        build_tree_warp<2>(s, st, s.bltree, sh_cnt);
        for (max_blindex = kBlCodes - 1; max_blindex >= 3; max_blindex--)
            if (s.bltree[bl_order(max_blindex)].dl != 0) break;
        if (lane == 0) st.opt_len += 3 * ((uint64_t)max_blindex + 1) + 5 + 5 + 4;
        __syncwarp();
        opt_lenb = (st.opt_len + 3 + 7) >> 3;
        static_lenb = (st.static_len + 3 + 7) >> 3;
        if (static_lenb <= opt_lenb || strategy_fixed) opt_lenb = static_lenb;
    }
    __syncwarp();
    if ((uint64_t)b.in_len + 4 <= opt_lenb && have_window) {
        if (lane == 0) { b.type = 0; b.hdr[0] = (uint8_t)b.last; b.hdr_bits = 3; b.body_bits = 0; }
    } else if (static_lenb == opt_lenb) {
        if (lane == 0) { b.type = 1; b.hdr[0] = (uint8_t)(2 | b.last); b.hdr_bits = 3; b.body_bits = st.static_len; }
        for (int n = (int)lane; n < kLCodes; n += 32) { b.lcode[n] = c_tab.sl_code[n]; b.llen[n] = c_tab.sl_len[n]; }
        if (lane < (uint32_t)kDCodes) { b.dcode[lane] = c_tab.sd_code[lane]; b.dlen[lane] = 5; }
    } else {
        if (lane == 0) {
            b.type = 2;
            WordSink o{b.hdr, 0};
            o.put(4 | b.last, 3);
            const int lcodes = lmax + 1, dcodes = dmax + 1, blcodes = max_blindex + 1;
            o.put((uint32_t)(lcodes - 257), 5);
            o.put((uint32_t)(dcodes - 1), 5);
            o.put((uint32_t)(blcodes - 4), 4);
            for (int r = 0; r < blcodes; r++) o.put(s.bltree[bl_order(r)].dl, 3);
            send_tree_fast(o, s.bltree, s.ltree, lcodes - 1);
            send_tree_fast(o, s.bltree, s.dtree, dcodes - 1);
            b.hdr_bits = o.nbits;
            b.body_bits = 3 + st.opt_len - o.nbits;
        }
        for (int n = (int)lane; n < kLCodes; n += 32) { b.lcode[n] = n <= lmax ? s.ltree[n].fc : 0; b.llen[n] = n <= lmax ? (uint8_t)s.ltree[n].dl : 0; }
        if (lane < (uint32_t)kDCodes) { b.dcode[lane] = (int)lane <= dmax ? s.dtree[lane].fc : 0; b.dlen[lane] = (int)lane <= dmax ? (uint8_t)s.dtree[lane].dl : 0; }
    }
    __syncwarp();
}

__global__ void __launch_bounds__(32) k_build_blocks(JobBufs jb, const uint32_t *freq)
{
    __shared__ TreeScratch s;
    __shared__ BlockDesc bd;
    __shared__ uint32_t fr[320];
    __shared__ uint32_t sh_cnt[16];
    __shared__ TreeState sh_st;
    const uint32_t b = blockIdx.x;
    if (b >= jb.info->n_blocks) return;
    for (uint32_t i = threadIdx.x; i < 320; i += 32) fr[i] = freq[b * 320 + i];
    for (uint32_t i = threadIdx.x; i < sizeof(BlockDesc) / 4; i += 32)
        reinterpret_cast<uint32_t *>(&bd)[i] = reinterpret_cast<const uint32_t *>(&jb.blocks[b])[i];
    __syncwarp();
    if (jb.serial_mode == 1) {
        if (threadIdx.x == 0) build_quick_piece(c_tab, bd, fr, fr + kLCodes, b == 0, b + 1 == jb.info->n_blocks, jb.not_last == 0);
    } else build_block_warp(s, bd, fr, fr + kLCodes, bd.have_window != 0, jb.strategy_fixed != 0, sh_cnt, &sh_st);
    __syncwarp();
    for (uint32_t i = threadIdx.x; i < sizeof(BlockDesc) / 4; i += 32)
        reinterpret_cast<uint32_t *>(&jb.blocks[b])[i] = reinterpret_cast<const uint32_t *>(&bd)[i];
}

__device__ __forceinline__ void or_bits(uint32_t *out32, uint64_t pos, uint64_t val, uint32_t n)
{
    if (n == 0) return;
    const uint64_t w = pos >> 5;
    const uint32_t sh = (uint32_t)(pos & 31);
    atomicOr(&out32[w], (uint32_t)(val << sh));
    if (sh + n > 32) {
        atomicOr(&out32[w + 1], (uint32_t)(val >> (32 - sh)));
        if (sh + n > 64) atomicOr(&out32[w + 2], (uint32_t)(val >> (64 - sh)));
    }
}

constexpr uint32_t kScanChunk = 1024;
__global__ void __launch_bounds__(256) k_scan_blocks(JobBufs jb)
{
    __shared__ uint64_t s_bits[kScanChunk];
    __shared__ uint64_t s_base[kScanChunk];
    __shared__ uint64_t s_bit;
    const uint32_t nb = jb.info->n_blocks;
    if (threadIdx.x == 0) s_bit = 8ull * jb.hdr_len + jb.prime_bits;
    for (uint32_t c0 = 0; c0 < nb; c0 += kScanChunk) {
        const uint32_t nc = min(kScanChunk, nb - c0);
        for (uint32_t i = threadIdx.x; i < nc; i += blockDim.x) {
            const BlockDesc &bd = jb.blocks[c0 + i];
            s_bits[i] = bd.type == 0 ? (1ull << 63) | (uint16_t)bd.in_len : (uint64_t)bd.hdr_bits + bd.body_bits;
        }
        __syncthreads();
        if (threadIdx.x == 0) {
            uint64_t bit = s_bit;
            for (uint32_t i = 0; i < nc; i++) {
                s_base[i] = bit;
                const uint64_t v = s_bits[i];
                bit = (v >> 63) ? ((bit + 3 + 7) & ~7ull) + 32 + 8ull * (v & 0xffffu) : bit + v;
            }
            s_bit = bit;
        }
        __syncthreads();
        for (uint32_t i = threadIdx.x; i < nc; i += blockDim.x) jb.blocks[c0 + i].bit_base = s_base[i];
        __syncthreads();
    }
    if (threadIdx.x != 0) return;
    uint64_t bit = s_bit;
    if (jb.not_last && jb.end_mode == 0) {
        const uint64_t p = (bit + 3 + 7) & ~7ull;
        jb.info->marker_byte = p >> 3;
        bit = p + 32;
    } else if (jb.not_last && jb.end_mode == 1) {
        or_bits(reinterpret_cast<uint32_t *>(jb.out), bit, 2u, 10);
        bit += 10;
    }
    jb.info->total_bits = bit;
    const uint64_t bytes = (jb.not_last && jb.end_mode ? (bit >> 3) : ((bit + 7) >> 3)) + (jb.wrap == 1 ? 4 : jb.wrap == 2 ? 8 : 0);
    jb.info->out_bytes = bytes;
    jb.info->data_type = jb.blocks[0].sym_count ? jb.blocks[0].data_type : 2u;
    if (bytes > jb.out_cap) { atomicOr(&jb.info->error, 8u); return; }
    if (jb.wrap == 1) {
        const uint32_t lf = (jb.huffman_only || jb.strategy_fixed || jb.level < 2) ? 0 : jb.level < 6 ? 1 : jb.level == 6 ? 2 : 3;
        uint32_t h = ((8u + (jb.cinfo << 4)) << 8) | (lf << 6);
        h += 31 - (h % 31);
        jb.out[0] = (uint8_t)(h >> 8);
        jb.out[1] = (uint8_t)h;
    } else if (jb.wrap == 2) {
        const uint8_t g[10] = {31, 139, 8, 0, 0, 0, 0, 0, (uint8_t)jb.xfl, 3};
        for (int i = 0; i < 10; i++) jb.out[i] = g[i];
    }
}

__global__ void __launch_bounds__(1024) k_encode(JobBufs jb)
{
    __shared__ HuffTables st;
    __shared__ uint16_t s_lcode[kLCodes], s_dcode[kDCodes];
    __shared__ uint8_t s_llen[kLCodes], s_dlen[kDCodes];
    __shared__ uint64_t warp_sum[32];
    if (jb.info->error) return;
    const BlockDesc &bd = jb.blocks[blockIdx.x];
    uint32_t *out32 = reinterpret_cast<uint32_t *>(jb.out);
    const uint32_t tid = threadIdx.x;
    if (bd.type == 0) {
        const uint64_t p = ((bd.bit_base + 3 + 7) >> 3);
        const uint32_t sl = (uint16_t)bd.in_len;
        if (tid == 0) {
            or_bits(out32, bd.bit_base, bd.hdr[0] & 7u, 3);
            jb.out[p] = (uint8_t)sl;
            jb.out[p + 1] = (uint8_t)(sl >> 8);
            jb.out[p + 2] = (uint8_t)~sl;
            jb.out[p + 3] = (uint8_t)((~sl) >> 8);
        }
        for (uint32_t i = tid; i < sl; i += blockDim.x) jb.out[p + 4 + i] = jb.in[bd.in_start + i];
        return;
    }
    for (uint32_t i = tid; i < sizeof(HuffTables) / 4; i += blockDim.x)
        reinterpret_cast<uint32_t *>(&st)[i] = reinterpret_cast<const uint32_t *>(&c_tab)[i];
    for (uint32_t i = tid; i < kLCodes; i += blockDim.x) { s_lcode[i] = bd.lcode[i]; s_llen[i] = bd.llen[i]; }
    if (tid < kDCodes) { s_dcode[tid] = bd.dcode[tid]; s_dlen[tid] = bd.dlen[tid]; }
    __syncthreads();
    for (uint32_t wi = tid; wi * 32 < bd.hdr_bits; wi += blockDim.x) {
        uint32_t v = bd.hdr[wi * 4] | (bd.hdr[wi * 4 + 1] << 8) | (bd.hdr[wi * 4 + 2] << 16) | ((uint32_t)bd.hdr[wi * 4 + 3] << 24);
        const uint32_t n = min(32u, bd.hdr_bits - wi * 32);
        if (n < 32) v &= (1u << n) - 1u;
        or_bits(out32, bd.bit_base + wi * 32ull, v, n);
    }
    const uint32_t total = bd.sym_count + (bd.no_eob ? 0u : 1u);
    const uint32_t lane = tid & 31, warp = tid >> 5;
    uint64_t round_bits = 0;
    for (uint32_t rb = 0; rb == 0 || rb < total; rb += blockDim.x * kSymsPerThread) {
        const uint32_t first = rb + tid * kSymsPerThread;
        uint64_t vals[kSymsPerThread];
        uint8_t lens[kSymsPerThread];
        uint32_t mybits = 0;
#pragma unroll
        for (uint32_t j = 0; j < kSymsPerThread; j++) {
            const uint32_t i = first + j;
            uint64_t v = 0;
            uint32_t n = 0;
            if (i < bd.sym_count) {
                const Sym s = jb.syms[bd.sym_begin + i];
                if (s.dist == 0) { v = s_lcode[s.lc]; n = s_llen[s.lc]; }
                else {
                    uint32_t code = st.length_code[s.lc];
                    v = s_lcode[code + 257];
                    n = s_llen[code + 257];
                    uint32_t extra = extra_lbits(code);
                    if (extra) { v |= (uint64_t)(s.lc - st.base_length[code]) << n; n += extra; }
                    const uint32_t d = s.dist - 1u;
                    code = st.dist_code[d < 256 ? d : 256 + (d >> 7)];
                    uint64_t dv = s_dcode[code];
                    uint32_t dn = s_dlen[code];
                    extra = extra_dbits(code);
                    if (extra) { dv |= (uint64_t)(d - st.base_dist[code]) << dn; dn += extra; }
                    v |= dv << n;
                    n += dn;
                }
            } else if (i + 1 == total && !bd.no_eob) { v = s_lcode[kEndBlock]; n = s_llen[kEndBlock]; }
            vals[j] = v;
            lens[j] = (uint8_t)n;
            mybits += n;
        }
        uint64_t incl = mybits;
#pragma unroll
        for (int o = 1; o < 32; o <<= 1) {
            const uint64_t t = __shfl_up_sync(0xffffffffu, incl, o);
            if ((int)lane >= o) incl += t;
        }
        if (lane == 31) warp_sum[warp] = incl;
        __syncthreads();
        if (warp == 0) {
            uint64_t ws = warp_sum[lane];
#pragma unroll
            for (int o = 1; o < 32; o <<= 1) {
                const uint64_t t = __shfl_up_sync(0xffffffffu, ws, o);
                if ((int)lane >= o) ws += t;
            }
            warp_sum[lane] = ws;
        }
        __syncthreads();
        uint64_t pos = bd.bit_base + bd.hdr_bits + round_bits + (incl - mybits) + (warp ? warp_sum[warp - 1] : 0);
#pragma unroll
        for (uint32_t j = 0; j < kSymsPerThread; j++) {
            or_bits(out32, pos, vals[j], lens[j]);
            pos += lens[j];
        }
        round_bits += warp_sum[31];
        __syncthreads();
    }
    if (tid == blockDim.x - 1 && round_bits != bd.body_bits) atomicOr(&jb.info->error, 16u);
}

__global__ void k_finish(JobBufs jb, const uint32_t *check)
{
    if (threadIdx.x != 0 || blockIdx.x != 0) return;
    if (jb.info->error) return;
    const uint64_t p = (jb.info->total_bits + 7) >> 3;
    const uint32_t a = *check;
    if (jb.not_last && jb.end_mode == 0) { jb.out[jb.info->marker_byte + 2] = 0xff; jb.out[jb.info->marker_byte + 3] = 0xff; }
    if (jb.wrap == 1) {
        jb.out[p] = (uint8_t)(a >> 24);
        jb.out[p + 1] = (uint8_t)(a >> 16);
        jb.out[p + 2] = (uint8_t)(a >> 8);
        jb.out[p + 3] = (uint8_t)a;
    } else if (jb.wrap == 2) {
        for (int i = 0; i < 4; i++) jb.out[p + i] = (uint8_t)(a >> (8 * i));
        for (int i = 0; i < 4; i++) jb.out[p + 4 + i] = (uint8_t)((jb.N - jb.start) >> (8 * i));
    }
    jb.info->adler = a;
}

__global__ void __launch_bounds__(256) k_literal_syms(JobBufs jb)
{
    const uint32_t p = blockIdx.x * blockDim.x + threadIdx.x;
    const uint32_t n = jb.N - jb.start;
    if (p == 0) {
        jb.info->n_mid_syms = n;
        jb.info->n_syms = n;
        jb.info->n_blocks = n / jb.block_syms + 1;
        const uint32_t w = jb.wsize, q = jb.N ? jb.N - 1 : 0;
        uint32_t B = q < 2 * w ? 0 : w * (1 + (q - 2 * w) / w);
        if (jb.N - B >= 2 * w - kMinLookahead) B += w;
        jb.info->final_base = B;
    }
    if (p < n) jb.syms[p] = Sym{0, jb.in[jb.start + p], jb.start + p};
}

__global__ void __launch_bounds__(256) k_stored(JobBufs jb)
{
    const uint32_t N = jb.N - jb.start;
    const uint32_t nb = N == 0 ? 1 : (N + 65534) / 65535;
    const uint32_t b = blockIdx.x;
    if (b >= nb) return;
    const uint32_t start = b * 65535u;
    const uint32_t len = min(65535u, N - start);
    uint8_t *o = jb.out + jb.hdr_len + (uint64_t)b * (65535u + 5u);
    if (threadIdx.x == 0) {
        o[0] = b + 1 == nb ? 1 : 0;
        o[1] = (uint8_t)len;
        o[2] = (uint8_t)(len >> 8);
        o[3] = (uint8_t)~len;
        o[4] = (uint8_t)((~len) >> 8);
        if (b == 0) {
            jb.info->total_bits = 8ull * (jb.hdr_len + (uint64_t)N + 5ull * nb);
            jb.info->out_bytes = jb.hdr_len + (uint64_t)N + 5ull * nb + (jb.wrap == 1 ? 4 : jb.wrap == 2 ? 8 : 0);
            jb.info->data_type = 2;
            if (jb.wrap == 1) {
                uint32_t h = (8u + (jb.cinfo << 4)) << 8;
                h += 31 - (h % 31);
                jb.out[0] = (uint8_t)(h >> 8);
                jb.out[1] = (uint8_t)h;
            }
            else if (jb.wrap == 2) {
                const uint8_t g[10] = {31, 139, 8, 0, 0, 0, 0, 0, 4, 3};
                for (int i = 0; i < 10; i++) jb.out[i] = g[i];
            }
        }
    }
    for (uint32_t i = threadIdx.x; i < len; i += blockDim.x) o[5 + i] = jb.in[jb.start + start + i];
}

__global__ void __launch_bounds__(256) k_links_dict_ghost(JobBufs jb, uint32_t *first)
{
    const uint32_t s = jb.start;
    if (s < 3 || s >= jb.N) return;
    const uint8_t *d = jb.in;
    const uint32_t g = s - 3;
    const uint32_t k0 = hash_u32((uint32_t)d[g] | ((uint32_t)d[g + 1] << 8) | ((uint32_t)d[g + 2] << 16));
    const uint32_t kt = hash_u32((uint32_t)d[g] | ((uint32_t)d[g + 1] << 8) | ((uint32_t)d[g + 2] << 16) | ((uint32_t)d[g + 3] << 24));
    if (k0 == kt) return;
    const uint32_t x = g + 1 + blockIdx.x * blockDim.x + threadIdx.x;
    if (x > g + kMaxDist || x + 4 > jb.N) return;
    const uint32_t kx = hash_u32((uint32_t)d[x] | ((uint32_t)d[x + 1] << 8) | ((uint32_t)d[x + 2] << 16) | ((uint32_t)d[x + 3] << 24));
    if (kx == k0) atomicMin(first, x);
}
__global__ void k_links_dict_ghost_apply(JobBufs jb, const uint32_t *first)
{
    if (threadIdx.x != 0 || blockIdx.x != 0) return;
    const uint32_t x = *first;
    if (x != 0xffffffffu) jb.L[x] = (uint16_t)(x - (jb.start - 3));
}

}
```

Baseline: 1.609.

## Use PDL launches, slim match smem, early-exit skip loop, add iter profiling

Launches the per-iteration parse kernels with programmatic dependent launch, so each kernel's launch overlaps the tail of the previous one. k_match stops copying the bucket map and diff bitmaps into shared memory; it reads them from global memory and keeps 16-bit prefix counts, which shrinks its smem footprint. The k_skip pointer-jumping loop drops warp words that are already finished, and the tail-tile special case and the larger match_sub sizes are removed. A per-iteration profiling table and API are added, and reading diff data from global memory may cost extra latency.

```diff
diff --git a/include/zb_engine.h b/include/zb_engine.h
--- a/include/zb_engine.h
+++ b/include/zb_engine.h
@@ -90,6 +90,7 @@
 
 ZB_API void zb_engine_set_profile(zb_engine *e, int on);
 ZB_API int zb_engine_get_profile(zb_engine *e, float *ms, uint32_t *launches, int n);
+ZB_API int zb_engine_get_iter_profile(zb_engine *e, float *rows, int max_iters);
 
 ZB_API void *zb_device_alloc(zb_engine *e, size_t bytes);
 ZB_API void zb_device_free(zb_engine *e, void *p);
diff --git a/zlib_rs_b200/__init__.py b/zlib_rs_b200/__init__.py
--- a/zlib_rs_b200/__init__.py
+++ b/zlib_rs_b200/__init__.py
@@ -95,6 +95,8 @@
         L.zb_crc32.argtypes = [vp, u32, vp, sz, ci, ctypes.POINTER(u32), ctypes.POINTER(ctypes.c_float)]
         L.zb_engine_set_profile.argtypes = [vp, ci]
         L.zb_engine_get_profile.argtypes = [vp, ctypes.POINTER(ctypes.c_float), ctypes.POINTER(u32), ci]
+        if hasattr(L, "zb_engine_get_iter_profile"):
+            L.zb_engine_get_iter_profile.argtypes = [vp, ctypes.POINTER(ctypes.c_float), ci]
         L.zb_device_alloc.argtypes, L.zb_device_alloc.restype = [vp, sz], vp
         L.zb_device_free.argtypes = [vp, vp]
         L.zb_copy_to_device.argtypes = [vp, vp, vp, sz]
@@ -363,5 +365,13 @@
         k = lib().zb_engine_get_profile(self.h, ms, ln, 12)
         return {self.PHASES[i]: {"ms": ms[i], "launches": ln[i]} for i in range(min(k, len(self.PHASES)))}
 
+    ITER_COLS = ["dirty_tiles", "path_tiles", "skip", "match", "nxt", "path", "holes", "lists", "host_gap"]
+
+    def get_iter_profile(self, max_iters=64):
+        nc = len(self.ITER_COLS)
+        rows = (ctypes.c_float * (nc * max_iters))()
+        k = lib().zb_engine_get_iter_profile(self.h, rows, max_iters)
+        return [{c: rows[i * nc + j] for j, c in enumerate(self.ITER_COLS)} for i in range(k)]
+
     def fill_random(self, dptr, n, seed=42):
         self._check(lib().zb_device_fill_random(self.h, dptr, n, seed))
diff --git a/zlib_rs_b200/csrc/zb_engine.cu b/zlib_rs_b200/csrc/zb_engine.cu
--- a/zlib_rs_b200/csrc/zb_engine.cu
+++ b/zlib_rs_b200/csrc/zb_engine.cu
@@ -10,10 +10,24 @@
 namespace zb {
 
 constexpr uint32_t kSlowSub9 = 24576;
-constexpr uint32_t kTailTiles = 2;
-constexpr uint32_t kTailSub = 512;
 
 thread_local char g_err[256] = "";
+
+template <typename... P, typename... A>
+static cudaError_t launch_pdl(void (*kernel)(P...), uint32_t grid, uint32_t block, size_t smem, cudaStream_t s, A... args)
+{
+    cudaLaunchAttribute at[1];
+    at[0].id = cudaLaunchAttributeProgrammaticStreamSerialization;
+    at[0].val.programmaticStreamSerializationAllowed = 1;
+    cudaLaunchConfig_t c = {};
+    c.gridDim = dim3(grid);
+    c.blockDim = dim3(block);
+    c.dynamicSmemBytes = smem;
+    c.stream = s;
+    c.attrs = at;
+    c.numAttrs = 1;
+    return cudaLaunchKernelEx(&c, kernel, args...);
+}
 
 static void set_err(const char *what, cudaError_t e)
 {
@@ -58,7 +72,7 @@
 __global__ void k_links_dict_ghost(JobBufs, uint32_t *);
 __global__ void k_links_dict_ghost_apply(JobBufs, const uint32_t *);
 
-constexpr uint32_t kMatchSmemBytes = (kWSize + kMatchSub + 512) + (kWSize + kMatchSub) * 2 + ((kWSize + kMatchSub) / 32 + 1) * 4 * 4 + 8192;
+constexpr uint32_t kMatchSmemBytes = (kWSize + kMatchSub + 512) + (kWSize + kMatchSub) * 2 + ((kWSize + kMatchSub) / 32 + 1) * 2 * 2;
 constexpr uint32_t kPathSmemBytes = kPathTile * 4 * 3;
 constexpr uint32_t kLinks2SmemBytes = 65536 * 2 + kLinkTile * 2 + kLinkTile + 64 + 2048;
 constexpr uint32_t kSkipSmemBytes = 2 * kWSize * 2 + 2 * (2 * kWSize / 32) * 4 + 8192 + 64;
@@ -129,19 +143,22 @@
 void Engine::pbegin()
 {
     if (!profile) return;
-    if (!pev0) { cudaEventCreate(&pev0); cudaEventCreate(&pev1); }
+    if (!pev0) { cudaEventCreate(&pev0); cudaEventCreate(&pev1); cudaEventCreate(&pevg); }
     cudaEventRecord(pev0, st);
 }
 
-void Engine::pend(int phase, uint32_t nlaunch)
+void Engine::pend(int phase, uint32_t nlaunch, int icol)
 {
     if (!profile) return;
     cudaEventRecord(pev1, st);
     cudaEventSynchronize(pev1);
     float ms = 0;
     cudaEventElapsedTime(&ms, pev0, pev1);
-    phase_ms[phase] += ms;
-    phase_launches[phase] += nlaunch;
+    if (phase >= 0) {
+        phase_ms[phase] += ms;
+        phase_launches[phase] += nlaunch;
+    }
+    if (icol >= 0 && prof_iters >= 1 && prof_iters <= (uint32_t)kIterProf) iter_prof[prof_iters - 1][icol] += ms;
 }
 
 int Engine::reserve(int slot, size_t bytes, void **out)
@@ -270,13 +287,13 @@
     uint32_t *d_mark_list = d_mark_cnt + 4;
     auto launch_chain = [&](uint32_t first_tile) {
         if (chain2) {
-            k_path_groups<<<chain_groups, 1024, chainG * kPathHead * 8, st>>>(jb, npt, chainG, d_gfn, d_mark_cnt);
-            k_path_chain2<<<chain_groups, 1024, chain2_smem, st>>>(jb, npt, chainG, d_gfn, d_mark_list, d_mark_cnt);
+            launch_pdl(k_path_groups, chain_groups, 1024, chainG * kPathHead * 8, st, jb, npt, chainG, d_gfn, d_mark_cnt);
+            launch_pdl(k_path_chain2, chain_groups, 1024, chain2_smem, st, jb, npt, chainG, d_gfn, d_mark_list, d_mark_cnt);
             launches++;
         } else k_path_chain<<<1, 1024, kChainSmemBytes, st>>>(jb, npt, first_tile);
     };
     auto launch_mark = [&](uint32_t grid) {
-        if (chain2) k_path_mark<<<grid < npt ? grid : npt, 1024, kPathSmemBytes, st>>>(jb, d_mark_list, d_mark_cnt);
+        if (chain2) launch_pdl(k_path_mark, grid < npt ? grid : npt, 1024, kPathSmemBytes, st, jb, (const uint32_t *)d_mark_list, (const uint32_t *)d_mark_cnt);
         else k_path_mark<<<npt, 1024, kPathSmemBytes, st>>>(jb, nullptr, nullptr);
     };
     uint32_t *d_lists;
@@ -355,7 +372,11 @@
     if (lf_zero && !jb.strategy_fixed && !jb.huffman_only) jb.level = 1;
 
     CK(cudaEventRecord(ev0, st));
-    if (profile) { for (int i = 0; i < kPhases; i++) { phase_ms[i] = 0; phase_launches[i] = 0; } }
+    if (profile) {
+        for (int i = 0; i < kPhases; i++) { phase_ms[i] = 0; phase_launches[i] = 0; }
+        memset(iter_prof, 0, sizeof iter_prof);
+        prof_iters = 0;
+    }
     uint32_t up_chunks = 0;
     size_t up_len[kUpChunks] = {0};
     const bool chunked_upload = !src_dev && !dstart && n_in >= ((size_t)4 << 20) && level != 0 && !jb.huffman_only &&
@@ -482,12 +503,22 @@
                 uint32_t n_dirty = nmt;
                 for (;;) {
                     iters++;
-                    uint32_t mthreads = 1024;
+                    if (profile) {
+                        prof_iters = iters;
+                        if (iters <= (uint32_t)kIterProf) {
+                            iter_prof[iters - 1][0] = (float)n_dirty;
+                            iter_prof[iters - 1][1] = (float)(iters > 1 ? h_info->n_ptiles : npt);
+                            if (iters > 1) {
+                                cudaEventRecord(pev1, st);
+                                cudaEventSynchronize(pev1);
+                                cudaEventElapsedTime(&iter_prof[iters - 1][8], pevg, pev1);
+                            }
+                        }
+                    }
                     if (iters == 1) jb.match_sub = 4096;
-                    else if (n_dirty <= kTailTiles) { jb.match_sub = kTailSub; mthreads = 256; }
                     else {
                         const uint64_t per_cta = (uint64_t)n_dirty * kMatchTile / (4 * (uint64_t)device_sm_count());
-                        jb.match_sub = per_cta >= 8192 ? 8192 : per_cta >= 4096 ? 4096 : per_cta >= 2048 ? 2048 : 1024;
+                        jb.match_sub = per_cta >= 2048 ? 2048 : 1024;
                     }
                     uint32_t nsub = (N + jb.match_sub - 1) / jb.match_sub;
                     uint32_t n_ptiles = npt, first_ptile = 0;
@@ -501,33 +532,36 @@
                         nsub = (n_dirty ? n_dirty : 1) * (kMatchTile / jb.match_sub);
                         if (n_dirty) {
                             pbegin();
-                            k_skip<<<n_dirty, 1024, kSkipSmemBytes, st>>>(jb);
-                            pend(1, 1);
+                            CK(launch_pdl(k_skip, n_dirty, 1024, kSkipSmemBytes, st, jb));
+                            pend(1, 1, 2);
                             launches++;
                         }
                     }
                     const uint32_t msmem = (kWSize + jb.match_sub + 512) + (kWSize + jb.match_sub) * 2 +
-                                           (iters > 1 ? ((kWSize + jb.match_sub) / 32 + 1) * 4 * 4 + 8192 : 64);
+                                           (iters > 1 ? ((kWSize + jb.match_sub) / 32 + 1) * 2 * 2 : 64);
                     jb.use_bucket_map = iters > 1;
                     pbegin();
-                    k_match<<<nsub, mthreads, msmem, st>>>(jb);
-                    pend(1, 1);
+                    CK(launch_pdl(k_match, nsub, 1024, msmem, st, jb));
+                    pend(1, 1, 3);
                     if (profile && iters == 1) phase_ms[11] = phase_ms[1];
                     pbegin();
-                    k_nxt<<<n_ptiles * (kPathTile / 1024), 1024, 0, st>>>(jb);
-                    pend(2, 1);
+                    CK(launch_pdl(k_nxt, n_ptiles * (kPathTile / 1024), 1024, 0, st, jb));
+                    pend(2, 1, 4);
                     pbegin();
-                    k_path_tiles<<<n_ptiles, 1024, kPathSmemBytes, st>>>(jb);
+                    CK(launch_pdl(k_path_tiles, n_ptiles, 1024, kPathSmemBytes, st, jb));
                     launch_chain(first_ptile);
                     launch_mark(iters == 1 ? npt : 2 * n_ptiles + 16);
-                    pend(3, 3);
+                    pend(3, 3, 5);
                     pbegin();
-                    k_holes<<<(nlists * kLongPerSub + 255) / 256, 256, 0, st>>>(jb, nlists);
-                    k_holes_cmp<<<(nwords + 255) / 256, 256, 0, st>>>(jb, nwords, nmt);
-                    pend(4, 2);
+                    CK(launch_pdl(k_holes, (nlists * kLongPerSub + 255) / 256, 256, 0, st, jb, nlists));
+                    CK(launch_pdl(k_holes_cmp, (nwords + 255) / 256, 256, 0, st, jb, nwords, nmt));
+                    pend(4, 2, 6);
                     launches += 7;
-                    k_iter_lists<<<1, 1024, 0, st>>>(jb, d_lists, d_lists + nmt + 8, npt);
+                    pbegin();
+                    CK(launch_pdl(k_iter_lists, 1, 1024, 0, st, jb, d_lists, d_lists + nmt + 8, npt));
                     launches++;
+                    pend(-1, 0, 7);
+                    if (profile) cudaEventRecord(pevg, st);
                     CK(cudaMemcpyAsync(h_info, d_info, sizeof(JobInfo), cudaMemcpyDeviceToHost, st));
                     CK(cudaStreamSynchronize(st));
                     if (h_info->error) { snprintf(g_err, sizeof g_err, "engine error flags 0x%x (parse)", h_info->error); return ZB_E_INTERNAL; }
@@ -748,6 +782,15 @@
     return k;
 }
 
+int zb_engine_get_iter_profile(zb_engine *z, float *rows, int max_iters)
+{
+    if (!z) return 0;
+    const int n = (int)(z->e.prof_iters < (uint32_t)Engine::kIterProf ? z->e.prof_iters : (uint32_t)Engine::kIterProf);
+    const int k = n < max_iters ? n : max_iters;
+    if (rows) memcpy(rows, z->e.iter_prof, sizeof(float) * Engine::kIterCols * (size_t)k);
+    return k;
+}
+
 void *zb_device_alloc(zb_engine *z, size_t bytes)
 {
     if (!z) return nullptr;
diff --git a/zlib_rs_b200/csrc/zb_engine_internal.h b/zlib_rs_b200/csrc/zb_engine_internal.h
--- a/zlib_rs_b200/csrc/zb_engine_internal.h
+++ b/zlib_rs_b200/csrc/zb_engine_internal.h
@@ -32,9 +32,12 @@
     bool profile = false;
     float phase_ms[kPhases] = {0};
     uint32_t phase_launches[kPhases] = {0};
-    cudaEvent_t pev0 = nullptr, pev1 = nullptr;
+    static constexpr int kIterProf = 64, kIterCols = 9;
+    float iter_prof[kIterProf][kIterCols] = {};
+    uint32_t prof_iters = 0;
+    cudaEvent_t pev0 = nullptr, pev1 = nullptr, pevg = nullptr;
     void pbegin();
-    void pend(int phase, uint32_t nlaunch);
+    void pend(int phase, uint32_t nlaunch, int icol = -1);
 
     int init(int dev);
     int inflate_init();
diff --git a/zlib_rs_b200/csrc/zb_kernels.cu b/zlib_rs_b200/csrc/zb_kernels.cu
--- a/zlib_rs_b200/csrc/zb_kernels.cu
+++ b/zlib_rs_b200/csrc/zb_kernels.cu
@@ -184,9 +184,12 @@
 __global__ void __launch_bounds__(256) k_links_fix_std(JobBufs jb) { links_fix_body<false>(jb); }
 __global__ void __launch_bounds__(256) k_links_fix_roll(JobBufs jb) { links_fix_body<true>(jb); }
 
+__device__ __forceinline__ void pdl_enter() { asm volatile("griddepcontrol.wait;\n\tgriddepcontrol.launch_dependents;" ::: "memory"); }
+
 constexpr uint32_t kSkipSpan = 2 * kWSize;
 __global__ void __launch_bounds__(1024) k_skip(JobBufs jb)
 {
+    pdl_enter();
     extern __shared__ __align__(16) uint8_t smem[];
     uint16_t *sL = reinterpret_cast<uint16_t *>(smem);
     uint32_t *sh = reinterpret_cast<uint32_t *>(smem + kSkipSpan * 2);
@@ -227,6 +230,7 @@
     }
     __syncthreads();
     const uint32_t lane = tid & 31, warp = tid >> 5, nwords = (span + 31) / 32;
+    auto is_hole = [&](uint32_t t) { return ((sh[t >> 5] >> (t & 31)) & 1u) != 0; };
     uint32_t nz[2];
 #pragma unroll
     for (int h = 0; h < 2; h++) {
@@ -239,27 +243,24 @@
         for (int h = 0; h < 2; h++) {
             uint32_t m = nz[h];
             while (m) {
-                const uint32_t w = warp * 64 + (__ffs(m) - 1) + 32 * h;
+                const uint32_t b = __ffs(m) - 1;
                 m &= m - 1;
+                const uint32_t w = warp * 64 + b + 32 * h;
                 const uint32_t i = w * 32 + lane;
-                const bool on = (((sh[w] & sf[w]) >> lane) & 1u) && i < span;
-                for (int rep = 0; rep < 6; rep++) {
-                    bool c = false;
-                    if (on) {
-                        const uint32_t d = sL[i];
-                        if (d != 0 && d <= i) {
-                            const uint32_t t = i - d;
-                            if ((sh[t >> 5] >> (t & 31)) & 1u) {
-                                const uint32_t d2 = sL[t];
-                                sL[i] = (uint16_t)((d2 == 0 || d + d2 > md) ? 0u : d + d2);
-                                c = true;
-                            }
-                        }
+                bool more = (((sh[w] & sf[w]) >> lane) & 1u) && i < span;
+                uint32_t d = more ? sL[i] : 0u;
+                more = more && d != 0 && d <= i && is_hole(i - d);
+                for (int rep = 0; rep < 6 && __any_sync(0xffffffffu, more); rep++) {
+                    if (more) {
+                        const uint32_t d2 = sL[i - d];
+                        d = (d2 == 0 || d + d2 > md) ? 0u : d + d2;
+                        sL[i] = (uint16_t)d;
+                        ch = 1;
+                        more = d != 0 && d <= i && is_hole(i - d);
                     }
                     __syncwarp();
-                    if (!__any_sync(0xffffffffu, c)) break;
-                    ch = 1;
                 }
+                if (!__any_sync(0xffffffffu, more)) nz[h] &= ~(1u << b);
             }
         }
         if (!__syncthreads_or(ch)) break;
@@ -290,9 +291,9 @@
 enum { LS_IDLE = 0, LS_WALK = 1, LS_PEND = 2, LS_DONE = 3, LS_FIN = 4 };
 
 struct DiffMaps {
-    const uint32_t *del, *pdel;
-    const uint32_t *add, *padd;
-    __device__ __forceinline__ static bool any(const uint32_t *b, const uint32_t *p, uint32_t lo, uint32_t hi)
+    const uint32_t *del; const uint16_t *pdel;
+    const uint32_t *add; const uint16_t *padd;
+    __device__ __forceinline__ static bool any(const uint32_t *b, const uint16_t *p, uint32_t lo, uint32_t hi)
     {
         const uint32_t c_hi = p[hi >> 5] + __popc(b[hi >> 5] & ((1u << (hi & 31)) - 1u));
         const uint32_t c_lo = p[lo >> 5] + __popc(b[lo >> 5] & ((1u << (lo & 31)) - 1u));
@@ -308,8 +309,8 @@
     hi = __funnelshift_r(w1, w2, sh);
 }
 
-__device__ __forceinline__ void match_tile_fast(const JobBufs &jb, const uint8_t *sdata, const uint16_t *sL, const uint32_t *sbm,
-                                                const DiffMaps dm, uint32_t ws, uint32_t te, uint32_t *s_next)
+__device__ __forceinline__ void match_tile_fast(const JobBufs &jb, const uint8_t *sdata, const uint16_t *sL, const uint32_t *bm0,
+                                                const uint32_t *bm1, const DiffMaps dm, uint32_t ws, uint32_t te, uint32_t *s_next)
 {
     const bool filt = jb.use_bucket_map != 0;
     const uint32_t dbase = (uint32_t)__cvta_generic_to_shared(sdata);
@@ -454,7 +455,7 @@
                     bool skip = false;
                     if (filt) {
                         const uint32_t h = hash_u32(sld_u32u(dbase + xr));
-                        skip = !((sbm[h >> 5] >> (h & 31)) & 1u);
+                        skip = !(((bm0[h >> 5] | bm1[h >> 5]) >> (h & 31)) & 1u);
                         if (!skip) {
                             const uint32_t rdo = RDout[xr];
                             const bool on_budget = rdo != 0xffffu && (rdo & 0x8000u);
@@ -497,6 +498,7 @@
 
 __global__ void __launch_bounds__(1024, 2) k_match(JobBufs jb)
 {
+    pdl_enter();
     extern __shared__ __align__(16) uint8_t smem[];
     __shared__ uint32_t s_next;
     __shared__ __align__(8) unsigned long long s_mbar;
@@ -511,18 +513,17 @@
     const uint32_t data_bytes = kWSize + sub + 512;
     uint8_t *sdata = smem;
     uint16_t *sL = reinterpret_cast<uint16_t *>(smem + data_bytes);
-    uint32_t *sh = reinterpret_cast<uint32_t *>(smem + data_bytes + (kWSize + sub) * 2);
-    uint32_t *sbm = sh;
     const uint32_t wmax = (kWSize + sub) / 32 + 1;
-    uint32_t *sdel = sbm + 2048, *pdel = sdel + wmax, *sadd = pdel + wmax, *padd = sadd + wmax;
+    uint16_t *pdel = reinterpret_cast<uint16_t *>(smem + data_bytes + (kWSize + sub) * 2), *padd = pdel + wmax;
     __shared__ uint32_t s_wsum[32];
     const uint32_t N = jb.N;
     const uint32_t te = min(ts + sub, N);
     const uint32_t ws = ts >= kWSize ? ts - kWSize : 0;
     const uint32_t tid = threadIdx.x, nthr = blockDim.x;
+    const uint32_t mt = ts / kMatchTile;
+    const uint32_t *bm1 = jb.bucket_map + (size_t)mt * 2048, *bm0 = mt ? bm1 - 2048 : bm1;
+    const uint32_t *gadd = jb.hdiff + (ws >> 5), *gdel = jb.hdiff + jb.hdiff_words + (ws >> 5);
     if (jb.use_bucket_map) {
-        const uint32_t mt = ts / kMatchTile;
-        const uint32_t *bm1 = jb.bucket_map + (size_t)mt * 2048, *bm0 = mt ? bm1 - 2048 : bm1;
         int hit = 0;
         for (uint32_t x = ts + tid; x < te; x += nthr) {
             const uint8_t *q = jb.in + x;
@@ -534,18 +535,17 @@
             }
         }
         if (!__syncthreads_or(hit)) return;
-        for (uint32_t i = tid; i < 2048; i += nthr) sbm[i] = bm0[i] | bm1[i];
         const uint32_t nwd = (te - ws + 31) / 32;
         const uint32_t per = (nwd + 1 + nthr - 1) / nthr;
         const uint32_t wb = tid * per;
         const uint32_t lane_ = tid & 31, warp_ = tid >> 5;
         for (int which = 0; which < 2; which++) {
-            const uint32_t *src = which ? jb.hdiff : jb.hdiff + jb.hdiff_words;
-            uint32_t *bits = which ? sadd : sdel, *pre = which ? padd : pdel;
+            const uint32_t *bits = which ? gadd : gdel;
+            uint16_t *pre = which ? padd : pdel;
             uint32_t mine = 0;
             for (uint32_t k = 0; k < per; k++) {
                 const uint32_t w = wb + k;
-                if (w <= nwd) { const uint32_t v = w < nwd ? src[(ws >> 5) + w] : 0u; bits[w] = v; mine += __popc(v); }
+                if (w < nwd) mine += __popc(bits[w]);
             }
             uint32_t incl = mine;
 #pragma unroll
@@ -560,7 +560,7 @@
             for (uint32_t k = 0; k < warp_; k++) run += s_wsum[k];
             for (uint32_t k = 0; k < per; k++) {
                 const uint32_t w = wb + k;
-                if (w <= nwd) { pre[w] = run; run += __popc(bits[w]); }
+                if (w <= nwd) { pre[w] = (uint16_t)run; run += w < nwd ? __popc(bits[w]) : 0u; }
             }
         }
     }
@@ -609,7 +609,7 @@
     const long long t_1 = clock64();
     const LevelParams lp = jb.lp;
     if (!lp.early_exit) {
-        match_tile_fast(jb, sdata, sL, sbm, DiffMaps{sdel, pdel, sadd, padd}, ws, te, &s_next);
+        match_tile_fast(jb, sdata, sL, bm0, bm1, DiffMaps{gdel, pdel, gadd, padd}, ws, te, &s_next);
         __syncthreads();
         if (tid == 0) {
             const long long t_2 = clock64();
@@ -624,7 +624,7 @@
         uint32_t v = 0;
         if (jb.use_bucket_map && x + 4 <= N) {
             const uint32_t h = hash_u32(a.byte(x) | (a.byte(x + 1) << 8) | (a.byte(x + 2) << 16) | (a.byte(x + 3) << 24));
-            if (!((sbm[h >> 5] >> (h & 31)) & 1u)) continue;
+            if (!(((bm0[h >> 5] | bm1[h >> 5]) >> (h & 31)) & 1u)) continue;
         }
         if (x + kMSafe <= N) {
             Match m = jb.wsize == kWSize ? lm_walk(a, x, 0xffffffffu, lp) : lm_walk(a, x, 0xffffffffu, lp, DynWin{jb.wsize});
@@ -650,6 +650,7 @@
 
 __global__ void __launch_bounds__(1024) k_nxt(JobBufs jb)
 {
+    pdl_enter();
     constexpr uint32_t per = kPathTile / 1024;
     const uint32_t tile = jb.nxt_list ? jb.nxt_list[blockIdx.x / per] : blockIdx.x / per;
     if (!path_tile_dirty(jb, tile)) return;
@@ -726,6 +727,7 @@
 
 __global__ void __launch_bounds__(1024) k_path_tiles(JobBufs jb)
 {
+    pdl_enter();
     extern __shared__ __align__(16) uint8_t smem[];
     uint32_t *nx = reinterpret_cast<uint32_t *>(smem);
     uint32_t *ex = nx + kPathTile;
@@ -841,6 +843,7 @@
 
 __global__ void __launch_bounds__(1024) k_path_groups(JobBufs jb, uint32_t ntiles, uint32_t G, uint4 *gfn, uint32_t *mark_cnt)
 {
+    pdl_enter();
     if (blockIdx.x == 0 && threadIdx.x == 0) *mark_cnt = 0;
     extern __shared__ __align__(16) uint8_t smem[];
     uint2 *hd = reinterpret_cast<uint2 *>(smem);
@@ -857,6 +860,7 @@
 __global__ void __launch_bounds__(1024) k_path_chain2(JobBufs jb, uint32_t ntiles, uint32_t G, const uint4 *gfn, uint32_t *mark_list,
                                                         uint32_t *mark_cnt)
 {
+    pdl_enter();
     extern __shared__ __align__(16) uint8_t smem[];
     uint2 *hd = reinterpret_cast<uint2 *>(smem);
     uint4 *sg = reinterpret_cast<uint4 *>(smem + (size_t)G * kPathHead * 8);
@@ -919,6 +923,7 @@
 
 __global__ void __launch_bounds__(1024) k_path_mark(JobBufs jb, const uint32_t *list, const uint32_t *list_cnt)
 {
+    pdl_enter();
     extern __shared__ __align__(16) uint8_t smem[];
     uint32_t *nx = reinterpret_cast<uint32_t *>(smem);
     uint32_t *ex = nx + kPathTile;
@@ -986,6 +991,7 @@
 
 __global__ void __launch_bounds__(256) k_holes(JobBufs jb, uint32_t nlists)
 {
+    pdl_enter();
     const uint32_t t = blockIdx.x * blockDim.x + threadIdx.x;
     {
         const uint32_t nthr = gridDim.x * blockDim.x;
@@ -1028,6 +1034,7 @@
 
 __global__ void __launch_bounds__(256) k_holes_cmp(JobBufs jb, uint32_t nwords, uint32_t nmtiles)
 {
+    pdl_enter();
     __shared__ uint32_t sb[2048];
     const uint32_t w = blockIdx.x * blockDim.x + threadIdx.x;
     uint32_t a = 0, b = 0;
@@ -1069,6 +1076,7 @@
 
 __global__ void __launch_bounds__(1024) k_iter_lists(JobBufs jb, uint32_t *skip_list, uint32_t *path_list, uint32_t npt)
 {
+    pdl_enter();
     __shared__ uint32_t s_wsum[32], s_total, s_first;
     const uint32_t tid = threadIdx.x, lane = tid & 31, warp = tid >> 5;
     if (tid == 0) s_first = 0xffffffffu;
```

Result: faster. 1.685 (median of 6 runs) (+4.7%).
